# pola-rs/polars

Hardware: AMD Instinct MI355X
Metric: rows/sec + achieved HBM GB/s, TPC-H Q1/Q3 SF100, 1/2/4/8 GPU vs CPU (higher is better)
Workload: dtype f64; 1 GPU; tpch_q1_sf100; rows_per_gpu=600000000, algorithmic_bytes_per_gpu_step=25200000000, parallelism=single GPU

## Files before the change

### include/polars_amd.h

```cpp
#ifndef POLARS_AMD_H
#define POLARS_AMD_H

#include <stddef.h>
#include <stdint.h>

#ifdef __cplusplus
extern "C" {
#endif

#define PLX_ABI_MAJOR 0
#define PLX_ABI_MINOR 1

#define PLX_OK 0
#define PLX_ERR_INVALID 1
#define PLX_ERR_HIP 2
#define PLX_ERR_UNSUPPORTED 3
#define PLX_ERR_OOM 4
#define PLX_ERR_SHAPE 5
#define PLX_ERR_NOT_FOUND 6
#define PLX_ERR_CANCELLED 7

typedef enum plx_dtype {
  PLX_BOOL = 0,
  PLX_I8 = 1,
// ... 213 lines not shown
  PLX_AE_BITMAP_LOOKUP = 12,
  PLX_AE_TEMPORAL = 13,
  PLX_AE_WINDOW = 14,
  PLX_AE_WINDOW_KEY = 15,
  PLX_AE_CUMULATIVE = 16,
  PLX_AE_RANK = 17
} plx_aexpr_kind;

typedef enum plx_operator {
  PLX_OP_EQ = 0, PLX_OP_NE = 1, PLX_OP_LT = 2, PLX_OP_LE = 3, PLX_OP_GT = 4, PLX_OP_GE = 5,
  PLX_OP_PLUS = 6, PLX_OP_MINUS = 7, PLX_OP_MULTIPLY = 8, PLX_OP_TRUE_DIVIDE = 9,
  PLX_OP_FLOOR_DIVIDE = 10, PLX_OP_MODULUS = 11, PLX_OP_AND = 12, PLX_OP_OR = 13, PLX_OP_XOR = 14
} plx_operator;

typedef struct plx_aexpr {
  int32_t kind;
  int32_t op;
  int32_t lhs;
  int32_t rhs;
  int32_t dtype;
  int32_t is_null;
  plx_scalar lit;
  const char* name;
  int32_t cond;
} plx_aexpr;

typedef enum plx_ir_kind {
  PLX_IR_SCAN = 0,
  PLX_IR_FILTER = 1,
  PLX_IR_SELECT = 2,
  PLX_IR_HSTACK = 3,
  PLX_IR_GROUPBY = 4,
  PLX_IR_JOIN = 5,
  PLX_IR_SORT = 6,
  PLX_IR_SLICE = 7,
  PLX_IR_DISTINCT = 8
} plx_ir_kind;

typedef enum plx_join_order {
  PLX_JOIN_ORDER_NONE = 0,
  PLX_JOIN_ORDER_LEFT = 1,
  PLX_JOIN_ORDER_RIGHT = 2,
  PLX_JOIN_ORDER_LEFT_RIGHT = 3,
  PLX_JOIN_ORDER_RIGHT_LEFT = 4
} plx_join_order;

typedef struct plx_ir {
  int32_t kind;
  int32_t input;
  int32_t input_right;
  int32_t predicate;
  plx_frame frame;
  const int32_t* exprs;
  int32_t n_exprs;
  const int32_t* keys;
  int32_t n_keys;
  const int32_t* keys_right;
  int32_t n_keys_right;
  int32_t how;
  int32_t maintain_order;
  const char* suffix;
  const uint8_t* sort_descending;
  const uint8_t* sort_nulls_last;
  int64_t slice_offset;
  int64_t slice_len;
  int32_t coalesce;
} plx_ir;

#define PLX_PLAN_NO_FUSION 1u
#define PLX_PLAN_NO_PARTITION 4u
#define PLX_PLAN_NO_DIRECT_JOIN 2u

int plx_execute_plan(const plx_ir* ir, int32_t n_ir, const plx_aexpr* exprs, int32_t n_exprs, int32_t root,
                     uint32_t flags, plx_frame* out);
int plx_describe_fusion(const plx_ir* ir, int32_t n_ir, const plx_aexpr* exprs, int32_t n_exprs, int32_t root, int32_t* fusable,
                        int32_t* static_shape_id, char* why_not, size_t why_cap);
int plx_debug_program_json(const plx_ir* ir, int32_t n_ir, const plx_aexpr* exprs, int32_t n_exprs, int32_t root, char* buf, size_t cap);
int plx_jit_selftest(const plx_ir* ir, int32_t n_ir, const plx_aexpr* exprs, int32_t n_exprs, int32_t root);
int plx_jit_stats(int32_t* compiled, double* compile_ms);
int plx_jit_set_min_rows(int64_t min_rows);
const char* plx_last_plan_description(void);
const char* plx_last_plan_encodings(void);
int32_t plx_last_scan_tile_rows(void);
int32_t plx_wide_tiles_choice(int32_t compiled, int32_t knob_on, int64_t n_rows, int32_t n_inputs, const int32_t* dtypes, const int32_t* nullable, const uint64_t* values,
                              const uint64_t* validity);

int plx_datagen_lineitem_q1(int64_t n_rows, uint64_t seed, plx_column* out_cols);
int plx_datagen_lineitem_q1_host(int64_t row0, int64_t n, uint64_t seed, int64_t* shipdate, uint8_t* returnflag, uint8_t* linestatus,
                                 int64_t* quantity, double* extendedprice, double* discount, double* tax);

int plx_datagen_orders_lineitem(int64_t n_orders, uint64_t seed, plx_column* out_orders, plx_column* out_lineitem);
int plx_datagen_orders_lineitem_host(int64_t order0, int64_t n, int64_t n_orders_total, uint64_t seed, int64_t* orderkey, int64_t* custkey,
                                     int64_t* orderdate, uint32_t* n_lines, int64_t line_cap, int64_t* l_orderkey, double* l_extendedprice,
                                     double* l_discount, int64_t* l_shipdate, int64_t* n_lines_out);
int plx_datagen_customer(int64_t n_customers, uint64_t seed, plx_column* out_cols);
int plx_datagen_customer_host(int64_t row0, int64_t n, uint64_t seed, int64_t* custkey, uint8_t* segment);
int plx_datagen_uniform(int32_t dtype, int64_t n_rows, uint64_t seed, uint32_t stream, int64_t lo, int64_t hi, double scale, plx_column* out);
int plx_datagen_uniform_host(int32_t dtype, int64_t row0, int64_t n, uint64_t seed, uint32_t stream, int64_t lo, int64_t hi, double scale, void* out);
int plx_datagen_zipf(int64_t n_rows, uint64_t seed, uint32_t stream, uint64_t x0_q62, int64_t n_keys, plx_column* out);
int plx_datagen_zipf_host(int64_t row0, int64_t n, uint64_t seed, uint32_t stream, uint64_t x0_q62, int64_t n_keys, int64_t* out);

typedef uint64_t plx_strdict;
int plx_strview_dict_encode(const void* views, const uint8_t* validity, int64_t bit_offset, int64_t n, const void* const* data_buffers, const int64_t* data_sizes,
                            int32_t n_data_buffers, plx_column* out_codes, plx_strdict* out_dict);
int plx_strview_dict_encode_device(plx_column views_u64_pairs, plx_column data_u8, plx_column* out_codes, plx_strdict* out_dict);
int plx_strview_stamp_nulls(plx_column views_u64_pairs, plx_column valid_bool);
int plx_strview_groupby(plx_column views_u64_pairs, plx_column value, plx_column* out_codes, plx_strdict* out_dict, plx_column* out_sum, plx_column* out_count, plx_column* out_len);
#define PLX_STR_MATCH_MAX_PATTERN 64
typedef enum plx_str_match_kind { PLX_STR_STARTS_WITH = 0, PLX_STR_ENDS_WITH = 1, PLX_STR_CONTAINS = 2 } plx_str_match_kind;
int plx_strdict_match(plx_strdict dict, int32_t kind, const uint8_t* pattern, int64_t pattern_len, plx_column* out_bool);
int plx_strview_match(plx_column views_u64_pairs, plx_column data_u8, int32_t kind, const uint8_t* pattern, int64_t pattern_len, plx_column* out_bool);
int plx_strview_match_host(const void* views, const uint8_t* data, int64_t data_len, int64_t n, int32_t kind, const uint8_t* pattern, int64_t pattern_len,
                           uint64_t* out_bits, uint64_t* out_valid);
int plx_bitmap_lookup(plx_column codes, plx_column lut_bool, plx_column* out_bool);
int plx_strdict_info(plx_strdict dict, int64_t* n_strings, int64_t* total_bytes);

typedef enum plx_time_unit { PLX_UNIT_DATE = 0, PLX_UNIT_MS = 1, PLX_UNIT_US = 2, PLX_UNIT_NS = 3 } plx_time_unit;
typedef enum plx_temporal_part_kind {
  PLX_PART_YEAR = 0, PLX_PART_MONTH = 1, PLX_PART_DAY = 2, PLX_PART_QUARTER = 3, PLX_PART_WEEKDAY = 4, PLX_PART_ORDINAL_DAY = 5,
  PLX_PART_HOUR = 6, PLX_PART_MINUTE = 7, PLX_PART_SECOND = 8, PLX_PART_DATE = 9
} plx_temporal_part_kind;
int plx_temporal_part(plx_column col, int part, int unit, plx_column* out);
int plx_temporal_part_host(const void* values, int unit, int part, int64_t n, void* out);

int plx_strdict_to_host(plx_strdict dict, int64_t* offsets, uint8_t* bytes);
int plx_strdict_free(plx_strdict dict);
int plx_datagen_id_views(int64_t n_rows, uint64_t seed, uint32_t stream, int64_t lo, int64_t hi, plx_column* out_views);
int plx_datagen_long_id_views(int64_t n_rows, uint64_t seed, uint32_t stream, int64_t lo, int64_t hi, plx_column* out_views, plx_column* out_data);

typedef uint64_t plx_parquet;
int plx_parquet_open(const char* path, plx_parquet* out);
int plx_parquet_close(plx_parquet file);
int plx_parquet_shape(plx_parquet file, int64_t* num_rows, int32_t* num_row_groups, int32_t* num_columns);
int plx_parquet_column_info(plx_parquet file, int32_t column, const char** name, int32_t* dtype, int32_t* logical, int32_t* nullable);
int plx_parquet_column_timezone(plx_parquet file, int32_t column, const char** timezone);
int plx_parquet_row_group_info(plx_parquet file, int32_t row_group, int64_t* num_rows, int64_t* compressed_bytes);
int plx_parquet_chunk_info(plx_parquet file, int32_t row_group, int32_t column, int32_t* codec, uint32_t* encodings, int64_t* compressed_bytes,
                           int64_t* uncompressed_bytes, int32_t* has_min_max, plx_scalar* min, plx_scalar* max, int64_t* null_count);
int plx_parquet_read(plx_parquet file, const int32_t* row_groups, int32_t n_row_groups, const int32_t* columns, int32_t n_columns, plx_frame* out);
int plx_parquet_categories(plx_parquet file, int32_t column, int64_t* n_strings, int64_t* total_bytes);
int plx_parquet_categories_to_host(plx_parquet file, int32_t column, int64_t* offsets, uint8_t* bytes);
int plx_parquet_column_strdict(plx_parquet file, int32_t column, plx_strdict* out);

typedef uint64_t plx_ipc;
int plx_ipc_open(const char* path, plx_ipc* out);
int plx_ipc_close(plx_ipc file);
int plx_ipc_shape(plx_ipc file, int64_t* num_rows, int32_t* num_batches, int32_t* num_columns);
int plx_ipc_column_info(plx_ipc file, int32_t column, const char** name, int32_t* dtype, int32_t* logical, int32_t* nullable);
int plx_ipc_column_timezone(plx_ipc file, int32_t column, const char** timezone);
int plx_ipc_batch_info(plx_ipc file, int32_t batch, int64_t* num_rows, int64_t* body_bytes, int32_t* compressed);
int plx_ipc_read(plx_ipc file, const int32_t* batches, int32_t n_batches, const int32_t* columns, int32_t n_columns, plx_frame* out);
int plx_ipc_read_string_views(plx_ipc file, const int32_t* batches, int32_t n_batches, int32_t column, plx_column* out_views, plx_column* out_data);
int plx_ipc_categories(plx_ipc file, int32_t column, int64_t* n_strings, int64_t* total_bytes);
int plx_ipc_categories_to_host(plx_ipc file, int32_t column, int64_t* offsets, uint8_t* bytes);
int plx_ipc_column_strdict(plx_ipc file, int32_t column, plx_strdict* out);

typedef uint64_t plx_comm;
int plx_comm_unique_id(uint8_t* out_128_bytes);
int plx_comm_init(const uint8_t* unique_id_128_bytes, int32_t rank, int32_t world_size, plx_comm* out);
int plx_comm_info(plx_comm comm, int32_t* rank, int32_t* world_size);
int plx_comm_free(plx_comm comm);
int plx_exchange_by_key(plx_comm comm, plx_frame frame, const char* key, uint64_t seed, plx_frame* out, uint64_t* rows_sent, uint64_t* bytes_sent);
int plx_allgather_frame(plx_comm comm, plx_frame frame, plx_frame* out);

typedef struct plx_profile_record {
  char name[48];
// ... 43 lines not shown
```

### polars_amd/_ffi.py

```python
from __future__ import annotations

import ctypes as C
import os
import threading
from typing import Optional

os.environ.setdefault("GPU_MAX_HW_QUEUES", "8")

_HERE = os.path.dirname(os.path.abspath(__file__))
LIB_PATH = os.path.join(_HERE, "libpolars_amd.so")

BOOL, I8, I16, I32, I64, U8, U16, U32, U64, F32, F64 = range(11)
EQ, NE, LT, LE, GT, GE = range(6)
ADD, SUB, MUL, TRUE_DIV, FLOOR_DIV, MOD = range(6)
AND, OR, XOR = range(3)
AGG_SUM, AGG_MEAN, AGG_MIN, AGG_MAX, AGG_COUNT, AGG_LEN, AGG_FIRST, AGG_VAR, AGG_STD = range(9)
AGG_QUANTILE = 9
AGG_N_UNIQUE = 10
UNIQUE_ANY, UNIQUE_FIRST, UNIQUE_LAST, UNIQUE_NONE = range(4)
UNIQUE_KEEPS = {"any": UNIQUE_ANY, "first": UNIQUE_FIRST, "last": UNIQUE_LAST, "none": UNIQUE_NONE}
QUANTILE_NEAREST, QUANTILE_LOWER, QUANTILE_HIGHER, QUANTILE_MIDPOINT, QUANTILE_LINEAR = range(5)
QUANTILE_INTERPOLATIONS = {"nearest": QUANTILE_NEAREST, "lower": QUANTILE_LOWER, "higher": QUANTILE_HIGHER, "midpoint": QUANTILE_MIDPOINT, "linear": QUANTILE_LINEAR}
JOIN_INNER, JOIN_LEFT, JOIN_SEMI, JOIN_ANTI, JOIN_FULL, JOIN_RIGHT = range(6)
JOIN_COALESCE_DEFAULT, JOIN_COALESCE, JOIN_KEEP_BOTH = range(3)
# ... 134 lines not shown
    "plx_parquet_chunk_info": (C.c_int, [C.c_uint64, C.c_int32, C.c_int32, _i32p, C.POINTER(C.c_uint32), _i64p, _i64p, _i32p, C.POINTER(Scalar), C.POINTER(Scalar), _i64p]),
    "plx_parquet_read": (C.c_int, [C.c_uint64, _i32p, C.c_int32, _i32p, C.c_int32, _u64p]),
    "plx_parquet_categories": (C.c_int, [C.c_uint64, C.c_int32, _i64p, _i64p]),
    "plx_parquet_categories_to_host": (C.c_int, [C.c_uint64, C.c_int32, C.c_void_p, C.c_void_p]),
    "plx_parquet_column_strdict": (C.c_int, [C.c_uint64, C.c_int32, _u64p]),
    "plx_ipc_open": (C.c_int, [C.c_char_p, _u64p]),
    "plx_ipc_close": (C.c_int, [C.c_uint64]),
    "plx_ipc_shape": (C.c_int, [C.c_uint64, _i64p, _i32p, _i32p]),
    "plx_ipc_column_info": (C.c_int, [C.c_uint64, C.c_int32, C.POINTER(C.c_char_p), _i32p, _i32p, _i32p]),
    "plx_ipc_column_timezone": (C.c_int, [C.c_uint64, C.c_int32, C.POINTER(C.c_char_p)]),
    "plx_ipc_batch_info": (C.c_int, [C.c_uint64, C.c_int32, _i64p, _i64p, _i32p]),
    "plx_ipc_read": (C.c_int, [C.c_uint64, _i32p, C.c_int32, _i32p, C.c_int32, _u64p]),
    "plx_ipc_read_string_views": (C.c_int, [C.c_uint64, _i32p, C.c_int32, C.c_int32, _u64p, _u64p]),
    "plx_ipc_categories": (C.c_int, [C.c_uint64, C.c_int32, _i64p, _i64p]),
    "plx_ipc_categories_to_host": (C.c_int, [C.c_uint64, C.c_int32, C.c_void_p, C.c_void_p]),
    "plx_ipc_column_strdict": (C.c_int, [C.c_uint64, C.c_int32, _u64p]),
    "plx_comm_unique_id": (C.c_int, [C.c_void_p]),
    "plx_comm_init": (C.c_int, [C.c_void_p, C.c_int32, C.c_int32, _u64p]),
    "plx_comm_info": (C.c_int, [C.c_uint64, C.POINTER(C.c_int32), C.POINTER(C.c_int32)]),
    "plx_comm_free": (C.c_int, [C.c_uint64]),
    "plx_exchange_by_key": (C.c_int, [C.c_uint64, C.c_uint64, C.c_char_p, C.c_uint64, _u64p, _u64p, _u64p]),
    "plx_allgather_frame": (C.c_int, [C.c_uint64, C.c_uint64, _u64p]),
    "plx_column_import_arrow": (C.c_int, [C.POINTER(ArrowArray), C.POINTER(ArrowSchema), _u64p]),
    "plx_column_import_series": (C.c_int, [C.POINTER(SeriesExport), _u64p]),
    "plx_column_export_arrow": (C.c_int, [C.c_uint64, C.POINTER(ArrowArray), C.POINTER(ArrowSchema)]),
    "plx_column_export_series": (C.c_int, [C.c_uint64, C.c_char_p, C.POINTER(SeriesExport)]),
    "plx_column_to_host": (C.c_int, [C.c_uint64, C.c_void_p, C.c_void_p, _i32p]),
    "plx_column_copy_to_device": (C.c_int, [C.c_uint64, C.c_void_p, C.c_void_p]),
    "plx_column_info": (C.c_int, [C.c_uint64, _i32p, _i64p, _i64p]),
    "plx_column_device_ptrs": (C.c_int, [C.c_uint64, C.POINTER(C.c_void_p), C.POINTER(C.c_void_p)]),
    "plx_column_retain": (C.c_int, [C.c_uint64]),
    "plx_column_free": (C.c_int, [C.c_uint64]),
    "plx_cmp": (C.c_int, [C.c_int, C.c_uint64, C.c_uint64, _u64p]),
    "plx_cmp_scalar": (C.c_int, [C.c_int, C.c_uint64, Scalar, _u64p]),
    "plx_bitmap_binop": (C.c_int, [C.c_int, C.c_uint64, C.c_uint64, _u64p]),
    "plx_bitmap_not": (C.c_int, [C.c_uint64, _u64p]),
    "plx_arith": (C.c_int, [C.c_int, C.c_uint64, C.c_uint64, _u64p]),
    "plx_arith_scalar": (C.c_int, [C.c_int, C.c_uint64, Scalar, C.c_int, _u64p]),
    "plx_cast": (C.c_int, [C.c_uint64, C.c_int, _u64p]),
    "plx_if_then_else": (C.c_int, [C.c_uint64, C.c_uint64, C.c_uint64, _u64p]),
    "plx_filter": (C.c_int, [C.c_uint64, C.c_uint64, _u64p]),
    "plx_gather": (C.c_int, [C.c_uint64, C.c_uint64, _u64p]),
    "plx_reduce": (C.c_int, [C.c_int, C.c_uint64, C.POINTER(Scalar), _i32p, _i32p]),
    "plx_reduce_var": (C.c_int, [C.c_uint64, C.c_int32, C.c_int32, C.POINTER(Scalar), _i32p, _i32p]),
    "plx_groupby_agg": (C.c_int, [_u64p, C.c_int32, _u64p, _i32p, C.c_int32, C.c_int32, _u64p, _u64p]),
    "plx_groupby_agg_ddof": (C.c_int, [_u64p, C.c_int32, _u64p, _i32p, C.c_int32, C.c_int32, _i32p, _u64p, _u64p]),
    "plx_reduce_quantile": (C.c_int, [C.c_uint64, C.c_double, C.c_int32, C.POINTER(Scalar), _i32p, _i32p]),
    "plx_groupby_agg_params": (C.c_int, [_u64p, C.c_int32, _u64p, _i32p, C.c_int32, C.c_int32, _i32p, C.POINTER(C.c_double), _i32p, _u64p, _u64p]),
    "plx_window_agg": (C.c_int, [_u64p, C.c_int32, _u64p, _i32p, C.c_int32, _i32p, C.POINTER(C.c_double), _i32p, _u64p]),
    "plx_cumulative": (C.c_int, [_u64p, C.c_int32, C.c_uint64, C.c_int32, C.c_int32, _u64p]),
    "plx_rank": (C.c_int, [_u64p, C.c_int32, C.c_uint64, C.c_int32, C.c_int32, _u64p]),
    "plx_join_indices": (C.c_int, [C.c_int, C.c_uint64, C.c_uint64, _u64p, _u64p]),
    "plx_datagen_lineitem_q1": (C.c_int, [C.c_int64, C.c_uint64, _u64p]),
    "plx_datagen_lineitem_q1_host": (C.c_int, [C.c_int64, C.c_int64, C.c_uint64, C.c_void_p, C.c_void_p, C.c_void_p, C.c_void_p, C.c_void_p, C.c_void_p, C.c_void_p]),
    "plx_datagen_orders_lineitem": (C.c_int, [C.c_int64, C.c_uint64, _u64p, _u64p]),
    "plx_datagen_orders_lineitem_host": (C.c_int, [C.c_int64, C.c_int64, C.c_int64, C.c_uint64, C.c_void_p, C.c_void_p, C.c_void_p, C.c_void_p, C.c_int64,
                                                   C.c_void_p, C.c_void_p, C.c_void_p, C.c_void_p, _i64p]),
    "plx_datagen_uniform": (C.c_int, [C.c_int32, C.c_int64, C.c_uint64, C.c_uint32, C.c_int64, C.c_int64, C.c_double, _u64p]),
    "plx_datagen_customer": (C.c_int, [C.c_int64, C.c_uint64, _u64p]),
    "plx_datagen_customer_host": (C.c_int, [C.c_int64, C.c_int64, C.c_uint64, C.c_void_p, C.c_void_p]),
    "plx_datagen_uniform_host": (C.c_int, [C.c_int32, C.c_int64, C.c_int64, C.c_uint64, C.c_uint32, C.c_int64, C.c_int64, C.c_double, C.c_void_p]),
    "plx_datagen_zipf": (C.c_int, [C.c_int64, C.c_uint64, C.c_uint32, C.c_uint64, C.c_int64, _u64p]),
    "plx_datagen_zipf_host": (C.c_int, [C.c_int64, C.c_int64, C.c_uint64, C.c_uint32, C.c_uint64, C.c_int64, C.c_void_p]),
    "plx_debug_program_json": (C.c_int, [C.POINTER(IR), C.c_int32, C.POINTER(AExpr), C.c_int32, C.c_int32, C.c_char_p, C.c_size_t]),
    "plx_reduce_n_unique": (C.c_int, [C.c_uint64, C.POINTER(C.c_uint32)]),
    "plx_distinct_mask": (C.c_int, [_u64p, C.c_int32, C.c_int32, _u64p]),
    "plx_sort_indices": (C.c_int, [_u64p, C.c_int32, C.POINTER(C.c_uint8), C.POINTER(C.c_uint8), C.c_int64, _u64p]),
    "plx_hash_partition": (C.c_int, [C.c_uint64, C.c_int32, C.c_uint64, _u64p, _i64p]),
    "plx_frame_new": (C.c_int, [C.POINTER(C.c_char_p), _u64p, C.c_int32, _u64p]),
    "plx_frame_free": (C.c_int, [C.c_uint64]),
    "plx_frame_concat": (C.c_int, [_u64p, C.c_int32, _u64p]),
    "plx_frame_shape": (C.c_int, [C.c_uint64, _i64p, _i32p]),
    "plx_frame_column": (C.c_int, [C.c_uint64, C.c_int32, C.POINTER(C.c_char_p), _u64p]),
    "plx_frame_dtypes": (C.c_int, [C.c_uint64, _i32p]),
    "plx_frame_to_host": (C.c_int, [C.c_uint64, C.POINTER(C.c_void_p), C.POINTER(C.c_void_p), _i32p]),
    "plx_execute_plan": (C.c_int, [C.POINTER(IR), C.c_int32, C.POINTER(AExpr), C.c_int32, C.c_int32, C.c_uint32, _u64p]),
    "plx_describe_fusion": (C.c_int, [C.POINTER(IR), C.c_int32, C.POINTER(AExpr), C.c_int32, C.c_int32, _i32p, _i32p, C.c_char_p, C.c_size_t]),
    "plx_jit_selftest": (C.c_int, [C.POINTER(IR), C.c_int32, C.POINTER(AExpr), C.c_int32, C.c_int32]),
    "plx_jit_stats": (C.c_int, [_i32p, C.POINTER(C.c_double)]),
    "plx_jit_set_min_rows": (C.c_int, [C.c_int64]),
    "plx_last_plan_description": (C.c_char_p, []),
    "plx_last_plan_encodings": (C.c_char_p, []),
    "plx_last_scan_tile_rows": (C.c_int32, []),
    "plx_wide_tiles_choice": (C.c_int32, [C.c_int32, C.c_int32, C.c_int64, C.c_int32, C.POINTER(C.c_int32), C.POINTER(C.c_int32), C.POINTER(C.c_uint64), C.POINTER(C.c_uint64)]),
    "plx_profile_enable": (C.c_int, [C.c_int]),
    "plx_profile_fetch": (C.c_int, [C.POINTER(ProfileRecord), C.c_int32, _i32p]),
    "plx_profile_clear": (C.c_int, []),
}

_lib: Optional[C.CDLL] = None


def lib() -> C.CDLL:
    global _lib
    if _lib is None:
        if not os.path.exists(LIB_PATH):
            raise ImportError(
                f"{LIB_PATH} is missing: build the HIP extension first "
                "(python -c 'import __graft_entry__ as g; g.build()' or make -C polars_amd/csrc). "
                "There is no CPU fallback in polars_amd.")
        l = C.CDLL(LIB_PATH, mode=C.RTLD_GLOBAL)
        for name, (res, args) in SIGNATURES.items():
            fn = getattr(l, name)
            fn.restype = res
            fn.argtypes = args
        _lib = l
    return _lib


def check(status: int) -> None:
    if status != 0:
        msg = lib().plx_last_error().decode("utf-8", "replace")
        if status == ERR_UNSUPPORTED:
            raise UnsupportedError(status, msg)
        raise PlxError(status, msg)


_initialised = False


def init(device: Optional[int] = None) -> None:
    global _initialised
    if device is None:
        device = int(os.environ.get("LOCAL_RANK", "0"))
    check(lib().plx_init(device))
    _initialised = True


def ensure_init() -> None:
    if not _initialised:
        init()


_tls = threading.local()


def set_plan_note(note) -> None:
    _tls.plan_note = note


def last_plan() -> str:
    note = getattr(_tls, "plan_note", None)
    return note if note is not None else lib().plx_last_plan_description().decode()


def last_plan_encodings() -> str:
    return lib().plx_last_plan_encodings().decode()


def last_scan_tile_rows() -> int:
    return int(lib().plx_last_scan_tile_rows())


def wide_tiles_choice(compiled, knob_on, n_rows, dtypes, nullable, values, validity) -> int:
    n = len(dtypes)
    return int(lib().plx_wide_tiles_choice(int(bool(compiled)), int(bool(knob_on)), int(n_rows), n, (C.c_int32 * n)(*[int(d) for d in dtypes]),
                                           (C.c_int32 * n)(*[int(bool(x)) for x in nullable]), (C.c_uint64 * n)(*[int(v) for v in values]), (C.c_uint64 * n)(*[int(v) for v in validity])))


def jit_set_min_rows(min_rows: int) -> None:
    check(lib().plx_jit_set_min_rows(int(min_rows)))


def encoded_set_decimal_min_rows(min_rows: int) -> None:
    check(lib().plx_encoded_set_decimal_min_rows(int(min_rows)))


def encoded_decimal_min_rows() -> int:
    return int(lib().plx_encoded_decimal_min_rows())


def jit_stats():
    n, ms = C.c_int32(), C.c_double()
    check(lib().plx_jit_stats(C.byref(n), C.byref(ms)))
    return n.value, ms.value
```

### polars_amd/csrc/abi.cpp

```cpp
#include <cstdio>
#include <cstring>
#include <memory>
#include <mutex>

#include "core.hpp"
#include "datagen_device.hpp"
#include "distinct.hpp"
#include "encoded_inputs.hpp"
#include "engine.hpp"
#include "fused_shapes.hpp"
#include "jit.hpp"
#include "join.hpp"
#include "kernels.hpp"
#include "kernels_fused.hpp"
#include "ops.hpp"
#include "cumulative.hpp"
#include "quantile.hpp"
#include "scan.hpp"
#include "sort.hpp"
#include "strmatch.hpp"
#include "temporal.hpp"

namespace plx {
void init_device(int ordinal);
// ... 1115 lines not shown
    if (n_lines) n_lines[j] = r.n_lines;
    const bool want_lines = l_orderkey || l_extendedprice || l_discount || l_shipdate;
    for (uint32_t q = 0; q < r.n_lines; q++, at++) {
      if (!want_lines) continue;
      PLX_REQUIRE(at < line_cap, PLX_ERR_INVALID, "datagen: line arrays too small");
      const datagen::Q3LineRow lr = datagen::q3_line_row(seed, (uint64_t)(order0 + j), q, r.orderdate);
      if (l_orderkey) l_orderkey[at] = r.orderkey;
      if (l_extendedprice) l_extendedprice[at] = lr.extendedprice;
      if (l_discount) l_discount[at] = lr.discount;
      if (l_shipdate) l_shipdate[at] = lr.shipdate;
    }
  }
  if (n_lines_out) *n_lines_out = at;
  PLX_CATCH
}
int plx_datagen_customer(int64_t n_customers, uint64_t seed, plx_column* out_cols) {
  PLX_TRY
  PLX_REQUIRE(n_customers >= 0 && out_cols, PLX_ERR_INVALID, "datagen: bad arguments");
  ColumnPtr k = make_column(PLX_I64, n_customers, false), sgm = make_column(PLX_U8, n_customers, false);
  k->null_count = 0; sgm->null_count = 0;
  k::datagen_customer(n_customers, seed, k->values->as<int64_t>(), sgm->values->as<uint8_t>());
  out_cols[0] = register_column(k); out_cols[1] = register_column(sgm);
  PLX_CATCH
}
int plx_datagen_customer_host(int64_t row0, int64_t n, uint64_t seed, int64_t* custkey, uint8_t* segment) {
  PLX_TRY
  PLX_REQUIRE(row0 >= 0 && n >= 0, PLX_ERR_INVALID, "datagen: bad arguments");
  for (int64_t j = 0; j < n; j++) {
    if (custkey) custkey[j] = row0 + j + 1;
    if (segment) segment[j] = datagen::customer_segment(seed, (uint64_t)(row0 + j + 1));
  }
  PLX_CATCH
}
int plx_datagen_uniform(int32_t dtype, int64_t n_rows, uint64_t seed, uint32_t stream_id, int64_t lo, int64_t hi, double scale, plx_column* out) {
  PLX_TRY
  PLX_REQUIRE(n_rows >= 0 && out && hi > lo && stream_id < 8, PLX_ERR_INVALID, "datagen: bad arguments");
  PLX_REQUIRE(dtype == PLX_I64 || dtype == PLX_U32 || dtype == PLX_F64, PLX_ERR_UNSUPPORTED, "datagen_uniform: dtype must be Int64, UInt32 or Float64");
  ColumnPtr c = make_column(dtype, n_rows, false); c->null_count = 0;
  k::datagen_uniform(dtype, n_rows, seed, stream_id, lo, hi, scale, c->values->ptr);
  *out = register_column(c);
  PLX_CATCH
}
int plx_datagen_uniform_host(int32_t dtype, int64_t row0, int64_t n, uint64_t seed, uint32_t stream_id, int64_t lo, int64_t hi, double scale, void* out) {
  PLX_TRY
  PLX_REQUIRE(row0 >= 0 && n >= 0 && (out || n == 0) && hi > lo && stream_id < 8, PLX_ERR_INVALID, "datagen: bad arguments");
  PLX_REQUIRE(dtype == PLX_I64 || dtype == PLX_U32 || dtype == PLX_F64, PLX_ERR_UNSUPPORTED, "datagen_uniform: dtype must be Int64, UInt32 or Float64");
  for (int64_t j = 0; j < n; j++) {
    const int64_t v = datagen::uniform_value(seed, stream_id, (uint64_t)(row0 + j), lo, hi);
    if (dtype == PLX_I64) reinterpret_cast<int64_t*>(out)[j] = v;
    else if (dtype == PLX_U32) reinterpret_cast<uint32_t*>(out)[j] = (uint32_t)v;
    else reinterpret_cast<double*>(out)[j] = (double)v * scale;
  }
  PLX_CATCH
}

int plx_datagen_zipf(int64_t n_rows, uint64_t seed, uint32_t stream_id, uint64_t x0_q62, int64_t n_keys, plx_column* out) {
  PLX_TRY
  PLX_REQUIRE(n_rows >= 0 && out && n_keys > 0 && stream_id < 8 && x0_q62 > 0 && x0_q62 < (1ull << 62), PLX_ERR_INVALID, "datagen_zipf: bad arguments");
  ColumnPtr c = make_column(PLX_I64, n_rows, false); c->null_count = 0;
  k::datagen_zipf(n_rows, seed, stream_id, x0_q62, n_keys, c->values->as<int64_t>());
  *out = register_column(c);
  PLX_CATCH
}
int plx_datagen_zipf_host(int64_t row0, int64_t n, uint64_t seed, uint32_t stream_id, uint64_t x0_q62, int64_t n_keys, int64_t* out) {
  PLX_TRY
  PLX_REQUIRE(row0 >= 0 && n >= 0 && (out || n == 0) && n_keys > 0 && stream_id < 8 && x0_q62 > 0 && x0_q62 < (1ull << 62), PLX_ERR_INVALID, "datagen_zipf: bad arguments");
  for (int64_t j = 0; j < n; j++) out[j] = datagen::zipf_value(seed, stream_id, (uint64_t)(row0 + j), x0_q62, n_keys);
  PLX_CATCH
}

int plx_execute_plan(const plx_ir* ir, int32_t n_ir, const plx_aexpr* exprs, int32_t n_exprs, int32_t root, uint32_t flags, plx_frame* out) {
  PLX_TRY
  PLX_REQUIRE(out, PLX_ERR_INVALID, "null out pointer");
  engine::Plan p = engine::import_plan(ir, n_ir, exprs, n_exprs, flags);
  FramePtr f = engine::execute(p, root);
  t_plan_desc = p.desc;
  t_plan_encoded = p.encoded;
  *out = register_frame(f);
  PLX_CATCH
}
const char* plx_last_plan_description(void) { return t_plan_desc.c_str(); }
const char* plx_last_plan_encodings(void) { return t_plan_encoded.c_str(); }
int32_t plx_last_scan_tile_rows(void) { return k::last_scan_tile_rows(); }
int32_t plx_wide_tiles_choice(int32_t compiled, int32_t knob_on, int64_t n_rows, int32_t n_inputs, const int32_t* dtypes, const int32_t* nullable, const uint64_t* values,
                              const uint64_t* validity) {
  if (n_inputs < 0 || n_inputs > fused::kMaxInputs || (n_inputs && (!dtypes || !nullable || !values || !validity))) return -1;
  fused::Shape sh{}; fused::Args args{};
  sh.n_inputs = (uint8_t)n_inputs; sh.pred = fused::kNone; sh.key = fused::kNone;
  args.n_rows = n_rows;
  for (int i = 0; i < n_inputs; i++) {
    sh.in_dtype[i] = (uint8_t)dtypes[i]; sh.in_nullable[i] = (uint8_t)(nullable[i] != 0);
    args.in[i].values = (const void*)(uintptr_t)values[i]; args.in[i].validity = (const uint64_t*)(uintptr_t)validity[i];
  }
  return k::wide_tiles_choice(sh, args, compiled != 0, knob_on != 0) ? 1 : 0;
}

int plx_debug_program_json(const plx_ir* ir, int32_t n_ir, const plx_aexpr* exprs, int32_t n_exprs, int32_t root, char* buf, size_t cap) {
  PLX_TRY
  PLX_REQUIRE(buf && cap > 0, PLX_ERR_INVALID, "null buffer");
  engine::Plan p = engine::import_plan(ir, n_ir, exprs, n_exprs, 0);
  std::string json, why;
  if (!engine::dump_program_json(p, root, &json, &why)) fail(PLX_ERR_UNSUPPORTED, "not a fusable pipeline: " + why);
  PLX_REQUIRE(json.size() + 1 <= cap, PLX_ERR_INVALID, "buffer too small for the program dump (" + std::to_string(json.size() + 1) + " bytes)");
  memcpy(buf, json.c_str(), json.size() + 1);
  PLX_CATCH
}

int plx_describe_fusion(const plx_ir* ir, int32_t n_ir, const plx_aexpr* exprs, int32_t n_exprs, int32_t root, int32_t* fusable, int32_t* static_shape_id,
                        char* why_not, size_t why_cap) {
  PLX_TRY
  engine::Plan p = engine::import_plan(ir, n_ir, exprs, n_exprs, 0);
  auto dump = [](const fused::Shape& sh) {
    std::string d = "inputs=" + std::to_string(sh.n_inputs) + " pred=" + std::to_string(sh.pred) + " key=" + std::to_string(sh.key) + " ops=[";
    for (int i = 0; i < sh.n_ops; i++) d += "(" + std::to_string(sh.ops[i].code) + "," + std::to_string(sh.ops[i].dst) + "," + std::to_string(sh.ops[i].a) + "," + std::to_string(sh.ops[i].b) + "," + std::to_string(sh.ops[i].c) + ")";
    d += "] aggs=[";
    for (int i = 0; i < sh.n_aggs; i++) d += "(" + std::to_string(sh.aggs[i].kind) + "," + std::to_string(sh.aggs[i].src) + ")";
    d += "] in_dtype=[";
    for (int i = 0; i < sh.n_inputs; i++) d += std::to_string(sh.in_dtype[i]) + (sh.in_nullable[i] ? "?" : "") + ",";
    d += "]";
    if (sh.n_keys) { d += " keys=["; for (int i = 0; i < sh.n_keys; i++) d += std::to_string(sh.keys[i]) + ","; d += "]"; }
    return d;
  };
  std::string why;
  int sid = -1;
  bool ok;
  PLX_REQUIRE(root >= 0 && root < (int)p.ir.size(), PLX_ERR_INVALID, "bad root");
  const engine::IRN& rn = p.ir[root];
  if (rn.kind == PLX_IR_GROUPBY && rn.input >= 0 && p.ir[rn.input].kind == PLX_IR_JOIN) {
    std::vector<fused::Shape> shapes;
    ok = engine::describe_join_fusion(p, root, &shapes, &why);
    if (ok) {
      sid = fused::find_static_shape(shapes[2]);
      t_plan_desc = dump(shapes[0]);
      for (size_t i = 1; i < shapes.size(); i++) t_plan_desc += "\n" + dump(shapes[i]);
    }
  } else {
    fused::Shape sh{};
    ok = engine::describe_fusion(p, root, &sh, &sid, &why);
    if (ok) t_plan_desc = dump(sh);
  }
  if (fusable) *fusable = ok ? 1 : 0;
  if (static_shape_id) *static_shape_id = sid;
  if (why_not && why_cap) snprintf(why_not, why_cap, "%s", why.c_str());
  PLX_CATCH
}

int plx_jit_selftest(const plx_ir* ir, int32_t n_ir, const plx_aexpr* exprs, int32_t n_exprs, int32_t root) {
  PLX_TRY
  engine::Plan p = engine::import_plan(ir, n_ir, exprs, n_exprs, 0);
  PLX_REQUIRE(root >= 0 && root < (int)p.ir.size(), PLX_ERR_INVALID, "bad root");
  const engine::IRN& rn = p.ir[root];
  std::string why;
  std::vector<std::pair<fused::Shape, jit::Sink>> jobs;
  if (rn.kind == PLX_IR_GROUPBY && rn.input >= 0 && p.ir[rn.input].kind == PLX_IR_JOIN) {
    std::vector<fused::Shape> shapes;
    PLX_REQUIRE(engine::describe_join_fusion(p, root, &shapes, &why), PLX_ERR_UNSUPPORTED, "not fusable: " + why);
    jobs = {{shapes[0], jit::REGAGG}, {shapes[1], jit::JOIN_BUILD}, {shapes[1], jit::DIRECT_BUILD}, {shapes[2], jit::PROBE_AGG}, {shapes[2], jit::DIRECT_PROBE}};
    for (size_t i = 3; i + 1 < shapes.size(); i++) jobs.push_back({shapes[i], jit::BITMAP_BUILD});
    for (uint32_t tiles : {2u, 4u}) jobs.push_back({shapes.back(), jit::part3_scatter_sink(fused::kP2Direct, tiles, fused::kPackRowid, false)});
  } else if (rn.kind == PLX_IR_FILTER) {
    fused::Shape sh{};
    PLX_REQUIRE(engine::describe_filter_fusion(p, root, &sh, &why), PLX_ERR_UNSUPPORTED, "not fusable: " + why);
    jobs = {{sh, jit::BALLOT}};
  } else {
    fused::Shape sh{}; int sid = -1;
    PLX_REQUIRE(engine::describe_fusion(p, root, &sh, &sid, &why), PLX_ERR_UNSUPPORTED, "not fusable: " + why);
    if (rn.kind == PLX_IR_SELECT) jobs = {{sh, jit::REGAGG}};
    else jobs = {{sh, jit::LDSAGG}, {sh, jit::DENSE}, {sh, jit::HASH}, {sh, jit::PART_COUNT}, {sh, jit::PART_SCATTER}, {sh, jit::PART_AGG},
                  {sh, jit::PART2_SCATTER_HASH}, {sh, jit::PART2_SCATTER_DIRECT}, {sh, jit::PART2_AGG_HASH}, {sh, jit::PART2_AGG_DIRECT},
                  {sh, jit::PART2_SCATTER_HASH_T2}, {sh, jit::PART2_SCATTER_DIRECT_T2}};
    if (rn.kind != PLX_IR_SELECT && sh.n_keys < 2) {
      for (uint32_t mode = 0; mode < 2; mode++) {
        const uint32_t best = fused::best_static_pack(sh, mode);
        for (uint32_t pack = 0; pack <= best; pack++) {
          if (pack == fused::kPackNarrow && fused::rec_layout2(sh, mode, fused::kPackNarrow).rec_words == fused::rec_layout2(sh, mode, fused::kPackNone).rec_words) continue;
          for (uint32_t tiles : {1u, 2u, 3u, 4u}) { jobs.push_back({sh, jit::part3_scatter_sink(mode, tiles, pack, false)}); jobs.push_back({sh, jit::part3_scatter_sink(mode, tiles, pack, true)}); }
          jobs.push_back({sh, jit::part3_agg_sink(mode, pack)});
        }
      }
      for (uint32_t mode = 0; mode < 2; mode++) {
        if (!fused::pair_pack_ok(sh, mode)) continue;
        for (uint32_t tiles : {1u, 2u, 3u, 4u}) { if (mode == fused::kP2Hash && tiles > 3) continue; jobs.push_back({sh, jit::part3_scatter_sink(mode, tiles, fused::kPackPair, false)}); jobs.push_back({sh, jit::part3_scatter_sink(mode, tiles, fused::kPackPair, true)}); }
        jobs.push_back({sh, jit::part3_agg_sink(mode, fused::kPackPair)});
      }
      if (fused::pairv_pack_ok(sh, fused::kP2Hash)) {
        for (uint32_t tiles : {1u, 2u, 3u}) { jobs.push_back({sh, jit::part3_scatter_sink(fused::kP2Hash, tiles, fused::kPackPairV, false)}); jobs.push_back({sh, jit::part3_scatter_sink(fused::kP2Hash, tiles, fused::kPackPairV, true)}); }
        jobs.push_back({sh, jit::part3_agg_sink(fused::kP2Hash, fused::kPackPairV)});
      }
    }
    if (sh.n_keys >= 2) {
      jobs = {{sh, jit::WIDE}};
      for (uint32_t pack = 0; pack <= std::min<uint32_t>(fused::best_static_pack(sh, fused::kP2Hash), fused::kPackNarrow); pack++) {
        for (uint32_t tiles : {1u, 2u, 3u}) jobs.push_back({sh, jit::part3_scatter_sink(fused::kP2Hash, tiles, pack, false)});
        jobs.push_back({sh, jit::part3_agg_sink(fused::kP2Hash, pack)});
      }
    }
  }
  {
    std::vector<std::pair<fused::Shape, jit::Sink>> forms;
    fused::Args aligned{}; aligned.n_rows = fused::kWideTileRows;
    for (auto& j : jobs) {
      const bool wide = k::wide_tiles_choice(j.first, aligned, true, true);
      if (j.second == jit::REGAGG && wide) forms.push_back({j.first, jit::REGAGG_WIDE});
      if (j.second == jit::LDSAGG && wide) forms.push_back({j.first, jit::LDSAGG_WIDE});
    }
    jobs.insert(jobs.end(), forms.begin(), forms.end());
  }
  for (auto& j : jobs) {
    const std::string log = jit::selftest(j.first, j.second);
    if (!log.empty()) fail(PLX_ERR_INVALID, "jit selftest failed: " + log.substr(0, 4000));
  }
  PLX_CATCH
}
int plx_jit_set_min_rows(int64_t min_rows) { PLX_TRY jit::set_min_rows(min_rows); PLX_CATCH }
int plx_jit_stats(int32_t* compiled, double* compile_ms) {
  PLX_TRY
  int c = 0; double ms = 0;
  jit::stats(&c, &ms);
  if (compiled) *compiled = c;
  if (compile_ms) *compile_ms = ms;
  PLX_CATCH
}

extern "C++" {
namespace {
struct StrDict { Buf views, data, offsets, bytes; int64_t n = 0; uint64_t total = 0; bool materialised = false; };
std::mutex g_strdict_mu;
std::vector<std::unique_ptr<StrDict>> g_strdicts;
StrDict& get_strdict(uint64_t h) {
  std::lock_guard<std::mutex> lk(g_strdict_mu);
  if (h == 0 || h > g_strdicts.size() || !g_strdicts[h - 1]) fail(PLX_ERR_INVALID, "invalid string dictionary handle");
  return *g_strdicts[h - 1];
}
uint64_t register_strdict(std::unique_ptr<StrDict> d) { std::lock_guard<std::mutex> lk(g_strdict_mu); g_strdicts.push_back(std::move(d)); return (uint64_t)g_strdicts.size(); }
void materialise(StrDict& d) {
  if (d.materialised) return;
  k::strdict_materialise(d.views->as<uint64_t>(), d.data ? d.data->as<uint8_t>() : nullptr, d.n, &d.offsets, &d.bytes, &d.total);
  d.materialised = true;
}
void encode_on_device(const uint64_t* views, const ColumnPtr& validity_holder, Buf data, Buf buf_base, int64_t n, plx_column* out_codes, plx_strdict* out_dict, bool from_stamps = false) {
  Buf codes, dviews, svalid;
  int64_t nd = 0, snulls = 0;
  k::strview_dict_encode(views, validity_holder ? validity_holder->valid_words() : nullptr, data ? data->as<uint8_t>() : nullptr, buf_base ? buf_base->as<uint64_t>() : nullptr, n, &codes, &dviews, &nd,
                         from_stamps && !validity_holder ? &svalid : nullptr, &snulls);
  auto c = std::make_shared<Column>();
  c->dtype = PLX_U32; c->len = n; c->values = codes;
  if (validity_holder && validity_holder->validity) c->validity = validity_holder->validity;
  else if (snulls > 0) { c->validity = svalid; c->null_count = snulls; }
  else c->null_count = 0;
  if (nd > 0) { c->range_state = 1; c->range_min = 0; c->range_max = nd - 1; c->range_trusted = true; }
  auto d = std::make_unique<StrDict>();
  d->views = dviews; d->data = data; d->n = nd;
  *out_codes = register_column(c);
  *out_dict = register_strdict(std::move(d));
}
}
namespace plx {
void strview_encode_device(const uint64_t* views, const ColumnPtr& validity_holder, Buf data, int64_t n, plx_column* out_codes, plx_strdict* out_dict) {
  Buf bb = dev_alloc_zero(8);
  encode_on_device(views, validity_holder, data, bb, n, out_codes, out_dict);
}
void strview_encode_device_bases(const uint64_t* views, const ColumnPtr& validity_holder, Buf data, Buf buf_base, int64_t n, plx_column* out_codes, plx_strdict* out_dict) {
  encode_on_device(views, validity_holder, data, buf_base, n, out_codes, out_dict);
}
}
}

int plx_strview_dict_encode(const void* views, const uint8_t* validity, int64_t bit_offset, int64_t n, const void* const* data_buffers, const int64_t* data_sizes,
                            int32_t n_data_buffers, plx_column* out_codes, plx_strdict* out_dict) {
  PLX_TRY
  PLX_REQUIRE(out_codes && out_dict && n >= 0 && (views || n == 0) && n_data_buffers >= 0 && (n_data_buffers == 0 || (data_buffers && data_sizes)), PLX_ERR_INVALID, "strview_dict_encode: bad arguments");
  device();
  Buf dv = dev_alloc((size_t)std::max<int64_t>(n, 1) * 16);
  if (n) h2d_sync_pinned(dv->ptr, views, (size_t)n * 16);
  ColumnPtr vh;
  if (validity) {
    std::vector<uint8_t> zeros((size_t)n);
    vh = column_from_host(PLX_U8, zeros.data(), validity, bit_offset, n);
  }
  uint64_t total = 0;
  std::vector<uint64_t> base((size_t)std::max(n_data_buffers, 1), 0);
  for (int i = 0; i < n_data_buffers; i++) { base[i] = total; total += (uint64_t)data_sizes[i]; }
  Buf data = dev_alloc((size_t)total + 64), bb = dev_alloc(sizeof(uint64_t) * base.size());
  for (int i = 0; i < n_data_buffers; i++) {
    if (!data_sizes[i]) continue;
    if ((uint64_t)data_sizes[i] >= ((uint64_t)32 << 20)) h2d_sync_pinned((uint8_t*)data->ptr + base[i], data_buffers[i], (size_t)data_sizes[i]);
    else h2d_async((uint8_t*)data->ptr + base[i], data_buffers[i], (size_t)data_sizes[i]);
  }
  h2d_async(bb->ptr, base.data(), sizeof(uint64_t) * base.size());
  PLX_HIP(hipStreamSynchronize(stream()));
  encode_on_device(dv->as<uint64_t>(), vh, data, bb, n, out_codes, out_dict);
  PLX_CATCH
}
// ... 242 lines not shown
```

### polars_amd/csrc/engine.cpp

```cpp
#include "engine.hpp"

#include <algorithm>
#include <atomic>
#include <cmath>
#include <functional>
#include <memory>
#include <numeric>
#include <optional>
#include <set>
#include <sstream>

#include "cumulative.hpp"
#include "distinct.hpp"
#include "encoded_inputs.hpp"
#include "fused_shapes.hpp"
#include "jit.hpp"
#include "join.hpp"
#include "kernels.hpp"
#include "kernels_fused.hpp"
#include "ops.hpp"
#include "quantile.hpp"
#include "sort.hpp"
#include "temporal.hpp"
#include "variance.hpp"
// ... 1208 lines not shown
  }
  int64_t mn, mx;
  if (col->range_state == 1 && col->range_trusted && !col->range_assumed) { mn = col->range_min; mx = col->range_max; }
  else {
    const k::ReduceResult rr = k::reduce_all(col->dtype, col->data(), col->valid_words(), n);
    if (rr.n_valid == 0) return nullptr;
    mn = (int64_t)rr.minmax_lo; mx = (int64_t)rr.minmax_hi;
  }
  uint64_t g = 0;
  if (enc::affine_needs_gcd(mn, mx)) {
    if (col->dtype != PLX_I64) return nullptr;
    g = enc::affine_gcd(col->values->as<int64_t>(), col->valid_words(), n, mn);
  }
  const enc::AffineChoice ch = enc::choose_affine(mn, mx, g);
  if (!ch.ok || ch.width * 4 > dtype_width(col->dtype)) return nullptr;
  s->kind = EncodedShadow::kAffine; s->width = ch.width; s->base = ch.base; s->stride = ch.stride;
  s->codes = dev_alloc(groups * (size_t)ch.width);
  if (!enc::affine_encode(col->dtype, col->data(), col->valid_words(), n, ch.base, ch.stride, ch.width, s->codes->ptr)) return nullptr;
  return s;
}
static std::shared_ptr<EncodedShadow> encoded_shadow_for_scan(const ColumnPtr& col, bool may_build) {
  if (!encoded_inputs_enabled()) return nullptr;
  std::shared_ptr<EncodedShadow> s = std::atomic_load(&col->shadow);
  if (s && s->kind != EncodedShadow::kNone) return s;
  if (!may_build || (s && s->never_encode) || !col->values || !col->values->owned || col->len <= 0) return nullptr;
  if (col->dtype != PLX_I64 && col->dtype != PLX_F64 && col->dtype != PLX_I32 && col->dtype != PLX_U32) return nullptr;
  auto next = std::make_shared<EncodedShadow>();
  next->scans = (s ? s->scans : 0) + 1;
  if (next->scans >= 2) {
    std::shared_ptr<EncodedShadow> built;
    try { built = build_shadow(col); }
    catch (const Error& e) { if (e.code != PLX_ERR_OOM) throw; (void)hipGetLastError(); }
    if (built) { built->scans = next->scans; next = built; }
    else next->never_encode = true;
  }
  std::atomic_store(&col->shadow, next);
  return next->kind != EncodedShadow::kNone ? next : nullptr;
}
struct ScanProgram { Shape shape; Args args; int static_id; std::string note; };
static ScanProgram scan_program_with_encodings(const Compiler& c, bool may_build) {
  ScanProgram sp{c.shape, c.args, -1, ""};
  enc::InputEncoding e[kMaxInputs];
  bool any = false;
  for (int i = 0; i < c.shape.n_inputs; i++) {
    const ColumnPtr& col = c.cols[c.input_cols[i]];
    if (c.args.in[i].values != col->data() || c.args.n_rows != col->len) continue;
    const std::shared_ptr<EncodedShadow> s = encoded_shadow_for_scan(col, may_build);
    if (!s) continue;
    e[i].kind = s->kind; e[i].width = s->width; e[i].base = s->base; e[i].stride = s->stride;
    e[i].codes = s->codes ? s->codes->ptr : nullptr; e[i].dict = s->dict ? s->dict->as<unsigned long long>() : nullptr;
    any = true;
  }
  uint32_t taken = 0;
  if (any && enc::encode_program(c.shape, c.args, e, &sp.shape, &sp.args, &taken)) {
    sp.note = "encoded{";
    bool first = true;
    for (int i = 0; i < c.shape.n_inputs; i++) {
      if (!((taken >> i) & 1u)) continue;
      std::string name = "?";
      for (size_t j = 0; j < c.df->cols.size(); j++) if (c.df->cols[j] == c.cols[c.input_cols[i]]) name = c.df->names[j];
      sp.note += std::string(first ? "" : ",") + name + ":" + (e[i].kind == EncodedShadow::kDict ? "dict" : e[i].kind == EncodedShadow::kDecimal ? "decimal" : "affine") + std::to_string(8 * e[i].width);
      first = false;
    }
    sp.note += "}";
  }
  sp.static_id = find_static_shape(sp.shape);
  return sp;
}

namespace {
struct GroupByRun {
  Compiler& c; const KeyPlan& kp; const Shape& sh; const Args& args;
  const int len_idx, static_id;
  const bool may_partition;
  FusedAggResult& res; std::string& desc;
};
std::string scan_tag(int static_id, int64_t n_rows) { return std::string("fused_scan[") + jit::program_mode(static_id, n_rows) + "]+"; }

void finish_table(GroupByRun& q, const Buf& cells, int64_t G, const Buf& oob) {
  compact_into(nullptr, cells->as<uint64_t>(), G, -1, q.sh.n_aggs, q.len_idx, q.res);
  check_oob_flag(oob);
  q.res.key_valid = nullptr;
}
void lds_table(GroupByRun& q) {
  const int G = 1 << q.kp.total_bits;
  Buf cells = dev_alloc(sizeof(uint64_t) * (size_t)G * q.sh.n_aggs);
  Buf oob = untrusted_key_bounds(q.c) ? dev_alloc_zero(8) : nullptr;
  k::fused_lds_agg(q.sh, q.args, G, q.static_id, cells->as<uint64_t>(), oob ? oob->as<unsigned int>() : nullptr);
  q.desc += scan_tag(q.static_id, q.args.n_rows) + "lds_table(G=" + std::to_string(G) + ",copies=" + std::to_string(k::lds_agg_copies(G, q.sh.n_aggs)) + ")";
  finish_table(q, cells, G, oob);
}
void dense_hbm_table(GroupByRun& q) {
  const int64_t G = (int64_t)1 << q.kp.total_bits;
  Buf cells = dev_alloc(sizeof(uint64_t) * (size_t)(G + 1) * q.sh.n_aggs);
  k::init_agg_cells(cells->as<uint64_t>(), G + 1, q.sh);
  Buf oob = untrusted_key_bounds(q.c) ? dev_alloc_zero(8) : nullptr;
  DenseTable t; t.acc = cells->as<unsigned long long>(); t.key_min = 0; t.n_groups = G; t.oob = oob ? oob->as<unsigned int>() : nullptr;
  k::fused_dense_agg(q.sh, q.args, t, q.static_id);
  q.desc += scan_tag(q.static_id, q.args.n_rows) + "dense_hbm_table(G=" + std::to_string(G) + ")";
  finish_table(q, cells, G, oob);
}

enum PartKeys { kPackedIds , kKeysWithValidity, kWideWords };
void take_partitioned(GroupByRun& q, PartKeys keys, int64_t g, const Buf& ok, const Buf& okv, const Buf& oacc, int64_t stride, const std::string& pd) {
  FusedAggResult& res = q.res;
  res.n_groups = g; res.n_aggs = q.sh.n_aggs; res.acc = oacc;
  if (keys == kWideWords) { res.wide_words = ok; res.wide_valid = okv; res.wide_stride = stride; }
  else { res.packed_keys = ok; res.key_valid = keys == kKeysWithValidity ? okv : nullptr; }
  q.desc += scan_tag(q.static_id, q.args.n_rows) + pd;
}
bool partitioned_v1(GroupByRun& q, double est_groups, bool any_nullable, PartKeys keys) {
  PartitionPlan pp;
  if (!k::partition_plan(q.sh, est_groups, any_nullable, &pp)) return false;
  std::string pd;
  Buf ok, okv, oacc;
  const int64_t g = k::partitioned_agg(q.sh, q.args, pp, q.static_id, &ok, &okv, &oacc, &pd);
  if (g < 0) { q.desc += "lds-overflow+"; return false; }
  take_partitioned(q, keys, g, ok, okv, oacc, 0, pd);
  return true;
}
struct PartTry {
  double plan_for = 0;
  double fallback = 0;
  int packed_bits = -1;
  std::vector<uint64_t> hot;
  k::SrcRange ranges[kMaxSrc];
  k::SrcRange key_rng;
  ColumnPtr stat_col;
  int attempts = 3;
  bool grow_to_largest = false;
  PartKeys keys = kPackedIds;
};
bool partitioned_v2(GroupByRun& q, PartTry& t) {
  for (int attempt = 0; attempt < t.attempts; attempt++) {
    PartPlan2 p2;
    auto plan = [&](double groups) { return k::partition_plan2(q.sh, groups, t.packed_bits, q.len_idx, q.args.n_rows, (int)t.hot.size(), &p2, t.ranges, &t.key_rng); };
    if (!plan(t.plan_for) && !(attempt == 0 && t.fallback > 0 && plan(t.fallback))) return false;
    std::string pd;
    Buf ok, okv, oacc;
    int64_t key_range[2] = {1, 0}, stride = 0;
    const int64_t g = k::partitioned_agg2(q.sh, q.args, p2, q.static_id, t.hot, &ok, &okv, &oacc, &pd, t.stat_col ? key_range : nullptr, &stride);
    if (g >= 0) {
      if (t.stat_col && key_range[0] <= key_range[1]) { t.stat_col->range_state = 1; t.stat_col->range_min = key_range[0]; t.stat_col->range_max = key_range[1]; t.stat_col->range_trusted = true; pd += "+key_range_learned"; }
      if (p2.check_src) mark_sources_verified(q.c);
      if (t.keys == kKeysWithValidity) q.desc += "hot=" + std::to_string(t.hot.size()) + "+";
      take_partitioned(q, t.keys, g, ok, okv, oacc, stride, pd);
      return true;
    }
    if (g == -2) { q.desc += "v2-unavailable+"; return false; }
    q.desc += t.attempts == 1 ? "lds-overflow+" : "lds-overflow(P=" + std::to_string(1u << p2.log2_parts) + ")+";
    if (p2.log2_parts >= 9) return false;
    t.plan_for = std::max(t.plan_for * 2.0, t.grow_to_largest ? (double)((uint64_t)p2.n_slots << 9) * 0.8 : (double)((uint64_t)p2.n_slots << p2.log2_parts) * 1.01);
  }
  return false;
}

bool partitioned_packed_ids(GroupByRun& q) {
  const int bits = q.kp.total_bits;
  const int64_t n = q.args.n_rows;
  const double est = std::min((double)((uint64_t)1 << std::min(bits, 40)), (double)n);
  if (part_version() != 2) return partitioned_v1(q, est, false, kPackedIds);
  PartTry t;
  t.plan_for = est; t.packed_bits = bits; t.attempts = 1;
  if (hot_keys_enabled() || bits > 25) {
    double g_est = 1e18;
    const int64_t d = sample_keys_cached(plain_key_column(q.c, q.kp), q.sh, q.args, q.static_id, q.len_idx, kPartSampleRows, hot_keys_enabled() ? &t.hot : nullptr, &g_est, q.desc);
    if (d >= 0) t.plan_for = std::min(est, std::min(g_est, (double)n) * 1.3);
    q.desc += "sample(distinct=" + std::to_string(d) + ",hot=" + std::to_string(t.hot.size()) + ")+";
  }
  const double hint = q.c.plan.group_hint;
  if (hint > 0) { t.plan_for = std::min(est, hint * 1.02 + 64.0); q.desc += "groups<=" + std::to_string((int64_t)hint) + "(plan)+"; }
// ... 2118 lines not shown
```

### polars_amd/csrc/fused_sinks.hpp

```cpp
#pragma once
#include <type_traits>

#include "fused_device.hpp"

namespace plx {
namespace k {

struct RegAggSink {
  struct Params { unsigned long long* partials; };
  uint64_t acc[kMaxAggs];
  template <class S> __device__ __forceinline__ void init(const S& sh, const Params&) {
#pragma unroll
    for (int k = 0; k < kMaxAggs; k++) acc[k] = (k < sh.n_aggs) ? agg_identity_dev(sh.aggs[k].kind) : 0ull;
  }
  template <class S, class RF> __device__ __forceinline__ void consume(const S& sh, const RF& rf, const bool pass[kRows], int64_t row0, const Params&) {
#pragma unroll
    for (int r = 0; r < kRows; r++) {
#pragma unroll
      for (int k = 0; k < kMaxAggs; k++) {
        if (k < sh.n_aggs) {
          const Agg ag = sh.aggs[k];
          uint64_t v = rf.get(r, ag.src);
          bool valid = (rf.getv(ag.src) >> r) & 1;
          acc[k] = agg_combine(ag.kind, acc[k], agg_row_value(ag.kind, v, pass[r], valid, (uint64_t)(row0 + r)));
        }
      }
    }
  }
  template <class S> __device__ __forceinline__ void finish(const S& sh, const Params& p) {
    __shared__ uint64_t sh_acc[kBlock / 64][kMaxAggs];
    const int lane = lane_id(), wave = threadIdx.x >> 6;
#pragma unroll
    for (int k = 0; k < kMaxAggs; k++) {
      if (k < sh.n_aggs) {
        uint64_t x = acc[k];
#pragma unroll
        for (int m = 32; m >= 1; m >>= 1) x = agg_combine(sh.aggs[k].kind, x, shfl_xor_u64(x, m));
        if (lane == 0) sh_acc[wave][k] = x;
      }
    }
    __syncthreads();
    if ((int)threadIdx.x < sh.n_aggs) {
      const int k = threadIdx.x;
      uint64_t x = sh_acc[0][k];
      for (int w = 1; w < (int)(blockDim.x >> 6); w++) x = agg_combine(sh.aggs[k].kind, x, sh_acc[w][k]);
      p.partials[(size_t)blockIdx.x * kMaxAggs + k] = x;
    }
  }
};

struct LdsAggSink {
  struct Params {
    unsigned long long* partials;
    unsigned long long* global_acc;
    int n_groups;
    int copies;
    unsigned int* oob;
  };
  template <class S> __device__ __forceinline__ void init(const S& sh, const Params& p) {
    extern __shared__ unsigned long long lds_tbl[];
    const int cells = p.n_groups * sh.n_aggs;
    for (int i = threadIdx.x; i < cells * p.copies; i += blockDim.x) lds_tbl[i] = agg_identity_dev(sh.aggs[(i / p.copies) % sh.n_aggs].kind);
    __syncthreads();
  }
  template <class S, class RF> __device__ __forceinline__ void consume(const S& sh, const RF& rf, const bool pass[kRows], int64_t row0, const Params& p) {
    extern __shared__ unsigned long long lds_tbl[];
    const int copy = lane_id() & (p.copies - 1);
#pragma unroll
    for (int r = 0; r < kRows; r++) {
      if (!pass[r]) continue;
      const uint64_t gid64 = rf.get(r, sh.key);
      if (gid64 >= (uint64_t)p.n_groups) { if (p.oob) *p.oob = 1u; continue; }
      const uint32_t gid = (uint32_t)gid64;
      unsigned long long* cells = lds_tbl + (size_t)gid * sh.n_aggs * p.copies + copy;
#pragma unroll
      for (int k = 0; k < kMaxAggs; k++) {
        if (k < sh.n_aggs) {
          const Agg ag = sh.aggs[k];
          uint64_t v = rf.get(r, ag.src);
          bool valid = (rf.getv(ag.src) >> r) & 1;
          if ((ag.kind == AGG_SUM_F || ag.kind == AGG_SUM_I || ag.kind == AGG_COUNT) && !valid) continue;
          uint64_t x = agg_row_value(ag.kind, v, true, valid, (uint64_t)(row0 + r));
          lds_atomic_agg(ag.kind, cells + k * p.copies, x);
        }
      }
    }
  }
  template <class S> __device__ __forceinline__ void finish(const S& sh, const Params& p) {
    extern __shared__ unsigned long long lds_tbl[];
    __syncthreads();
    const int cells = p.n_groups * sh.n_aggs;
    for (int i = threadIdx.x; i < cells; i += blockDim.x) {
      const uint8_t kind = sh.aggs[i % sh.n_aggs].kind;
      uint64_t x = lds_tbl[(size_t)i * p.copies];
      for (int c = 1; c < p.copies; c++) x = agg_combine(kind, x, lds_tbl[(size_t)i * p.copies + c]);
      if (p.global_acc) { if (x != agg_identity_dev(kind) || kind == AGG_SUM_F) atomic_agg(kind, p.global_acc + i, x); }
      else p.partials[(size_t)blockIdx.x * cells + i] = x;
    }
  }
};

struct DenseAggSink {
  using Params = DenseTable;
  template <class S> __device__ __forceinline__ void init(const S&, const Params&) {}
  template <class S> __device__ __forceinline__ void finish(const S&, const Params&) {}
  template <class S, class RF> __device__ __forceinline__ void consume(const S& sh, const RF& rf, const bool pass[kRows], int64_t row0, const Params& p) {
#pragma unroll
    for (int r = 0; r < kRows; r++) {
      if (!pass[r]) continue;
      bool kvalid = (rf.getv(sh.key) >> r) & 1;
      int64_t g = kvalid ? ((int64_t)rf.get(r, sh.key) - p.key_min) : p.n_groups;
      if ((uint64_t)g > (uint64_t)p.n_groups || (kvalid && g == p.n_groups)) { if (p.oob) *p.oob = 1u; continue; }
      atomic_row(sh, rf, r, row0 + r, p.acc + (size_t)g * sh.n_aggs);
    }
  }
};

struct HashAggSink {
  using Params = HashTable;
  template <class S> __device__ __forceinline__ void init(const S&, const Params&) {}
  template <class S> __device__ __forceinline__ void finish(const S&, const Params&) {}
  __device__ __forceinline__ static int64_t find_slot(const Params& p, uint64_t key) {
    const uint64_t cap = 1ull << p.log2_cap;
    uint64_t slot = (key * 0x55fbfd6bfc5458e9ull) >> (64 - p.log2_cap);
    for (uint32_t probe = 0; probe < p.max_probe; probe++) {
      unsigned long long cur = p.keys[slot];
      if (cur == key) return (int64_t)slot;
      if (cur == kEmptyKey) {
        unsigned long long old = atomicCAS(&p.keys[slot], (unsigned long long)kEmptyKey, (unsigned long long)key);
        if (old == kEmptyKey || old == key) return (int64_t)slot;
      }
      slot = (slot + 1) & (cap - 1);
    }
    atomicExch(p.overflow, 1u);
    return -1;
  }
  static constexpr int kCombineRounds = 8;
  template <class S, class RF> __device__ __forceinline__ void consume_combined(const S& sh, const RF& rf, const bool pass[kRows], int64_t row0, const Params& p) {
    const uint64_t cap = 1ull << p.log2_cap;
    const int lane = lane_id();
#pragma unroll
    for (int r = 0; r < kRows; r++) {
      const bool kvalid = (rf.getv(sh.key) >> r) & 1;
      const uint64_t key = kvalid ? rf.get(r, sh.key) : 0ull;
      uint64_t xv[kMaxAggs];
#pragma unroll
      for (int k = 0; k < kMaxAggs; k++) {
        xv[k] = 0;
        if (k < sh.n_aggs) { const Agg ag = sh.aggs[k]; xv[k] = agg_row_value(ag.kind, rf.get(r, ag.src), true, (rf.getv(ag.src) >> r) & 1, (uint64_t)(row0 + r)); }
      }
      bool reached = false, keeps_total = false;
      uint64_t todo = ballot(pass[r]);
#pragma unroll 1
      for (int round = 0; round < kCombineRounds && todo; round++) {
        const int leader = (int)__builtin_ctzll(todo);
        const uint64_t lkey = shfl_u64(key, leader);
        const bool lvalid = __shfl((int)kvalid, leader, 64) != 0;
        const bool member = pass[r] && !reached && kvalid == lvalid && key == lkey;
        todo &= ~ballot(member);
#pragma unroll
        for (int k = 0; k < kMaxAggs; k++) {
          if (k < sh.n_aggs) {
            uint64_t x = member ? xv[k] : agg_identity_dev(sh.aggs[k].kind);
#pragma unroll
            for (int m = 32; m >= 1; m >>= 1) x = agg_combine(sh.aggs[k].kind, x, shfl_xor_u64(x, m));
            if (lane == leader) xv[k] = x;
          }
        }
        if (member) reached = true;
        if (lane == leader) keeps_total = true;
      }
      if (!pass[r] || (reached && !keeps_total)) continue;
      int64_t slot;
      if (!kvalid) { slot = (int64_t)cap; p.keys[cap] = 0; }
      else if (key == kEmptyKey) { slot = (int64_t)cap + 1; p.keys[cap + 1] = 0; }
      else slot = find_slot(p, key);
      if (slot < 0) continue;
#pragma unroll
      for (int k = 0; k < kMaxAggs; k++) {
        if (k < sh.n_aggs) {
          const uint8_t kind = sh.aggs[k].kind;
          if (xv[k] != agg_identity_dev(kind) || kind == AGG_SUM_F) atomic_agg(kind, p.acc + (size_t)slot * sh.n_aggs + k, xv[k]);
        }
// ... 238 lines not shown
};

struct BitmapBuildSink {
  using Params = BitmapBuild;
  unsigned long long n = 0;
  template <class S> __device__ __forceinline__ void init(const S&, const Params&) { n = 0; }
  template <class S> __device__ __forceinline__ void finish(const S&, const Params& p) {
    const uint64_t w = wave_sum_u64(n);
    if (lane_id() == 0 && w) atomicAdd(p.count, (unsigned long long)w);
  }
  template <class S, class RF> __device__ __forceinline__ void consume(const S& sh, const RF& rf, const bool pass[kRows], int64_t, const Params& p) {
#pragma unroll
    for (int r = 0; r < kRows; r++) {
      if (!pass[r] || !((rf.getv(sh.key) >> r) & 1)) continue;
      const uint64_t idx = rf.get(r, sh.key) - (uint64_t)p.kmin;
      if (idx >= p.range) continue;
      n++;
      __hip_atomic_fetch_or(&p.bits[idx >> 6], 1ull << (idx & 63), __ATOMIC_RELAXED, __HIP_MEMORY_SCOPE_AGENT);
    }
  }
};

struct DirectHitsSink {
  using Params = DirectHits;
  template <class S> __device__ __forceinline__ void init(const S&, const Params&) {}
  template <class S> __device__ __forceinline__ void finish(const S&, const Params&) {}
  template <class S, class RF> __device__ __forceinline__ void consume(const S& sh, const RF& rf, const bool pass[kRows], int64_t row0, const Params& p) {
    bool hit[kRows];
#pragma unroll
    for (int r = 0; r < kRows; r++) {
      bool ok = pass[r] && ((rf.getv(sh.key) >> r) & 1);
      const uint64_t idx = rf.get(r, sh.key) - (uint64_t)p.t.kmin;
      ok = ok && idx < p.t.range;
      if (ok) ok = (p.t.bits[idx >> 6] >> (idx & 63)) & 1ull;
      hit[r] = ok;
    }
    const unsigned long long b0 = ballot(hit[0]), b1 = ballot(hit[1]);
    if (lane_id() == 0) {
      const int64_t t = row0 / kTileRows;
      *reinterpret_cast<ulonglong2*>(p.out.ballots + t * 2) = make_ulonglong2(b0, b1);
      p.out.counts[t] = (unsigned int)(popc64(b0) + popc64(b1));
    }
  }
};

template <class P, bool FULL>
__device__ __forceinline__ void direct_probe_tile(const Args& args, const DirectJoinTable& p, int64_t base, RegFile& rf) {
  constexpr Shape sh = P::shape();
  const int64_t row0 = base + (int64_t)lane_id() * kRows;
  run_split<P, FULL, true>(args, row0, rf);
  if (!(p.opts & kDirectLateLoads)) run_split<P, FULL, false>(args, row0, rf);
  bool hit[kRows], any = false;
  unsigned long long slot[kRows];
#pragma unroll
  for (int r = 0; r < kRows; r++) {
    bool ok = FULL || (row0 + r < args.n_rows);
    if (sh.pred != kNone) ok = ok && (rf.get(r, sh.pred) & 1) && ((rf.getv(sh.pred) >> r) & 1);
    ok = ok && ((rf.getv(sh.key) >> r) & 1);
    const uint64_t idx = rf.get(r, sh.key) - (uint64_t)p.kmin;
    ok = ok && idx < p.range;
    slot[r] = 0;
    if (ok) {
      const unsigned long long w = p.bits[idx >> 6];
      ok = (w >> (idx & 63)) & 1ull;
      if (ok) slot[r] = direct_slot(p, idx, w);
    }
    hit[r] = ok; any = any || ok;
  }
  if (any) {
    if (p.opts & kDirectLateLoads) run_split<P, FULL, false>(args, row0, rf);
#pragma unroll
    for (int r = 0; r < kRows; r++)
      if (hit[r]) atomic_row(sh, rf, r, row0 + r, p.acc + (size_t)slot[r] * sh.n_aggs);
  }
}

template <class P, class Sink>
__host__ __device__ constexpr bool late_probe() {
  if constexpr (P::kStatic && std::is_same<Sink, DirectProbeAggSink>::value) return split_program(P::shape()).any_late;
  else return false;
}
template <class P, class Sink>
__host__ __device__ constexpr bool trust_nullable() {
  if constexpr (P::kStatic && (std::is_same<Sink, LdsAggSink>::value || std::is_same<Sink, RegAggSink>::value)) return narrow_rows(P::shape());
  else return false;
}
template <class P, class Sink>
__host__ __device__ constexpr bool wide_tiles_form() {
  if constexpr (trust_nullable<P, Sink>()) return wide_tiles_shape(P::shape());
  else return false;
}
template <class P, class Sink, bool WIDE = false>
__device__ __forceinline__ void fused_scan_body(const Shape dsh, const Args args, const typename Sink::Params sp) {
  Sink sink;
  typename RegFileOf<P>::type rf = make_regfile<P>(args);
  const int64_t wave = ((int64_t)blockIdx.x * blockDim.x + threadIdx.x) >> 6;
  const int64_t nwaves = ((int64_t)gridDim.x * blockDim.x) >> 6;
  const int64_t ntiles = (args.n_rows + kTileRows - 1) / kTileRows;
  if constexpr (late_probe<P, Sink>()) {
    for (int64_t t = wave; t < ntiles; t += nwaves) {
      const int64_t base = t * kTileRows;
      if (base + kTileRows <= args.n_rows) direct_probe_tile<P, true>(args, sp, base, rf);
      else direct_probe_tile<P, false>(args, sp, base, rf);
    }
  } else if constexpr (P::kStatic) {
    constexpr Shape sh = P::shape();
    constexpr int ND = dict_count(sh);
    constexpr bool kTrust = trust_nullable<P, Sink>();
    if constexpr (ND > 0) { stage_dicts<ND>(args); __syncthreads(); }
    sink.init(sh, sp);
    int64_t first_tile = 0;
    if constexpr (WIDE) {
      static_assert(wide_tiles_form<P, Sink>(), "wide tiles: a compiled aggregate scan over narrow rows without nullable inputs");
      const int64_t nwide = args.n_rows / kWideTileRows;
      const int lane = lane_id();
      for (int64_t t = wave; t < nwide; t += nwaves) {
        const int64_t row0 = t * kWideTileRows + (int64_t)lane * kWideRows;
        WideRaw raw;
        wide_load<P>(args, row0, raw);
#pragma unroll
        for (int j = 0; j < kWideRows / kRows; j++) {
          run_program_wide<P, ND>(args, raw, j, rf);
          bool pass[kRows];
#pragma unroll
          for (int r = 0; r < kRows; r++) pass[r] = sh.pred == kNone || ((rf.get(r, sh.pred) & 1) && ((rf.getv(sh.pred) >> r) & 1));
          sink.consume(sh, rf, pass, row0 + kRows * j, sp);
        }
      }
      first_tile = nwide * (kWideTileRows / kTileRows);
    }
    for (int64_t t = first_tile + wave; t < ntiles; t += nwaves) {
      bool pass[kRows]; int64_t row0;
      tile_rows<P, ND, kTrust>(dsh, args, t, rf, pass, row0);
      sink.consume(sh, rf, pass, row0, sp);
    }
    sink.finish(sh, sp);
  } else {
    sink.init(dsh, sp);
    for (int64_t t = wave; t < ntiles; t += nwaves) {
      bool pass[kRows]; int64_t row0;
      tile_rows<P>(dsh, args, t, rf, pass, row0);
      sink.consume(dsh, rf, pass, row0, sp);
    }
    sink.finish(dsh, sp);
  }
}

template <class P, class Sink>
__global__ __launch_bounds__(kBlock) void fused_scan_kernel(Shape dsh, Args args, typename Sink::Params sp) {
  fused_scan_body<P, Sink>(dsh, args, sp);
}
template <class P, class Sink>
__global__ __launch_bounds__(kBlock) void fused_scan_wide_kernel(Shape dsh, Args args, typename Sink::Params sp) {
  fused_scan_body<P, Sink, true>(dsh, args, sp);
}

struct BallotSink {
  using Params = BallotOut;
  template <class S> __device__ __forceinline__ void init(const S&, const Params&) {}
  template <class S> __device__ __forceinline__ void finish(const S&, const Params&) {}
  template <class S, class RF> __device__ __forceinline__ void consume(const S&, const RF&, const bool pass[kRows], int64_t row0, const Params& p) {
    const unsigned long long b0 = ballot(pass[0]), b1 = ballot(pass[1]);
    if (lane_id() == 0) {
      const int64_t t = row0 / kTileRows;
      *reinterpret_cast<ulonglong2*>(p.ballots + t * 2) = make_ulonglong2(b0, b1);
      p.counts[t] = (unsigned int)(popc64(b0) + popc64(b1));
    }
// ... 6 lines not shown
```

### polars_amd/csrc/jit.cpp

```cpp
#include "jit.hpp"

#include <dlfcn.h>
#include <sys/stat.h>
#include <unistd.h>
#include <hip/hip_runtime_api.h>
#include <hip/hiprtc.h>

#include <atomic>
#include <chrono>
#include <cstdlib>
#include <cstring>
#include <map>
#include <mutex>
#include <sstream>
#include <string>
#include <vector>

#include "core.hpp"
#include "kconfig.hpp"

namespace plx {
namespace jit {

using namespace fused;

namespace {
struct Entry { hipModule_t mod = nullptr; hipFunction_t fn = nullptr; bool failed = false; };
std::mutex g_mu;
std::map<std::string, Entry> g_cache;
int g_compiled = 0;
double g_ms = 0;

bool wide_tiles(Sink s) { return s == REGAGG_WIDE || s == LDSAGG_WIDE; }
const char* sink_type(Sink s) {
  static const char* n[] = {"RegAggSink", "LdsAggSink", "DenseAggSink", "HashAggSink", "WideAggSink", "JoinBuildSink", "ProbeAggSink", "DirectBuildSink", "DirectProbeAggSink", "BitmapBuildSink",
                            "part_count", "part_scatter", "part_agg", "part2_scatter_hash", "part2_scatter_direct", "part2_agg_hash", "part2_agg_direct", "part2_scatter_hash_t2", "part2_scatter_direct_t2"};
  if (s == REGAGG_WIDE) return "RegAggSink";
  if (s == LDSAGG_WIDE) return "LdsAggSink";
  if (s == PART3_AGG_PAIRV) return "part3_agg";
  if (s >= PART3_SCATTER_PAIRV && s < PART3_AGG_PAIRV) return "part3_scatter";
  if (s == PART3_AGG_PAIR || s == PART3_AGG_PAIR_DIRECT) return "part3_agg";
  if (s >= PART3_SCATTER_PAIR && s < PART3_AGG_PAIR) return "part3_scatter";
  if (s == BALLOT) return "BallotSink";
  if (s == DIRECT_HITS) return "DirectHitsSink";
  if (s >= PART3_AGG) return "part3_agg";
  if (s >= PART3_SCATTER) return "part3_scatter";
  return n[s];
}

std::string include_dir() {
  if (const char* e = getenv("PLX_JIT_INCLUDE")) return e;
  Dl_info info;
  if (dladdr((const void*)&stats, &info) && info.dli_fname) {
    std::string p = info.dli_fname;
    size_t k = p.rfind('/');
    return (k == std::string::npos ? std::string(".") : p.substr(0, k)) + "/csrc";
  }
  return "polars_amd/csrc";
}

std::string resource_include() {
  if (const char* e = getenv("PLX_JIT_CLANG_INCLUDE")) return e;
  const char* roots[] = {"/opt/rocm/lib/llvm/lib/clang", "/opt/rocm/llvm/lib/clang"};
  for (const char* r : roots) {
    for (int v = 30; v >= 14; v--) {
      const std::string p = std::string(r) + "/" + std::to_string(v) + "/include";
      if (FILE* f = fopen((p + "/stddef.h").c_str(), "r")) { fclose(f); return p; }
    }
  }
  return "/opt/rocm/lib/llvm/lib/clang/22/include";
}
std::vector<std::string> compile_options() {
  std::vector<std::string> o = {"--offload-arch=gfx950", "-O3", "-std=c++17", "-ffp-contract=off", "-munsafe-fp-atomics", "-Wno-pass-failed", "-ffreestanding",
                                "-I" + include_dir(), "-I/opt/rocm/include", "-I" + resource_include()};
  if (const char* e = getenv("PLX_JIT_DEFINES")) { std::istringstream is(e); std::string t; while (is >> t) if (t.compare(0, 2, "-D") == 0) o.push_back(t); }
  return o;
}

uint64_t fnv1a(const std::string& s, uint64_t h = 0xcbf29ce484222325ull) { for (unsigned char c : s) { h ^= c; h *= 0x100000001b3ull; } return h; }

std::string kernel_symbol(const Shape& sh, Sink sink) {
  std::string key((const char*)&sh, sizeof(Shape));
  key.push_back((char)sink);
  char out[96];
  snprintf(out, sizeof out, "plx_jit_%s_%d_%08x", sink_type(sink), (int)sink, (unsigned)(fnv1a(key) & 0xffffffffu));
  return out;
}

std::string source_for(const Shape& sh, Sink sink) {
  std::ostringstream o;
  const std::string sym = kernel_symbol(sh, sink);
  o << "#define plx_jit_kernel " << sym << "\n";
  o << ((sink == BALLOT || sink == DIRECT_HITS || wide_tiles(sink)) ? "#include \"fused_sinks.hpp\"\n" : sink >= PART3_SCATTER ? "#include \"partition3_device.hpp\"\n" : sink >= PART2_SCATTER_HASH ? "#include \"partition2_device.hpp\"\n" : sink >= PART_COUNT ? "#include \"partition_device.hpp\"\n" : "#include \"fused_sinks.hpp\"\n") << "namespace plx { namespace k {\n"
       "struct JitProg {\n  static constexpr bool kStatic = true; static constexpr int kId = -2;\n  static constexpr Shape shape() {\n    Shape s{};\n";
  o << "    s.n_inputs = " << (int)sh.n_inputs << "; s.n_ops = " << (int)sh.n_ops << "; s.n_aggs = " << (int)sh.n_aggs << "; s.pred = " << (int)sh.pred
    << "; s.key = " << (int)sh.key << "; s.n_keys = " << (int)sh.n_keys << ";\n";
  for (int i = 0; i < kMaxKeys; i++) o << "    s.keys[" << i << "] = " << (int)sh.keys[i] << ";\n";
  for (int i = 0; i < sh.n_inputs; i++) o << "    s.in_dtype[" << i << "] = " << (int)sh.in_dtype[i] << "; s.in_nullable[" << i << "] = " << (int)sh.in_nullable[i] << ";\n";
  for (int i = 0; i < sh.n_ops; i++)
    o << "    s.ops[" << i << "] = mkop(" << (int)sh.ops[i].code << ", " << (int)sh.ops[i].dst << ", " << (int)sh.ops[i].a << ", " << (int)sh.ops[i].b << ", " << (int)sh.ops[i].c << ");\n";
  for (int i = 0; i < sh.n_aggs; i++) o << "    s.aggs[" << i << "] = Agg{" << (int)sh.aggs[i].kind << ", " << (int)sh.aggs[i].src << "};\n";
  o << "    return s;\n  }\n};\n";
  switch (sink) {
    case PART_COUNT:
      o << "extern \"C\" __global__ __launch_bounds__(kBlock) void plx_jit_kernel(Shape dsh, Args args, uint32_t log2_parts, unsigned int* hist) {\n"
           "  part_count_body<JitProg>(dsh, args, log2_parts, hist);\n}\n}}\n";
      break;
    case PART_SCATTER:
      o << "extern \"C\" __global__ __launch_bounds__(kBlock) void plx_jit_kernel(Shape dsh, Args args, PartitionPlan pp, const unsigned long long* part_off, "
           "const unsigned long long* wg_prefix, unsigned long long* out) {\n  part_scatter_body<JitProg>(dsh, args, pp, part_off, wg_prefix, out);\n}\n}}\n";
      break;
    case PART_AGG:
      o << "extern \"C\" __global__ __launch_bounds__(kAggBlock) void plx_jit_kernel(Shape dsh, PartitionPlan pp, PartAggParams ap) {\n"
           "  constexpr Shape csh = JitProg::shape(); constexpr RecLayout cl = rec_layout(JitProg::shape());\n  part_agg_body(csh, cl, pp, ap);\n}\n}}\n";
      break;
    case PART2_SCATTER_HASH: case PART2_SCATTER_DIRECT: case PART2_SCATTER_HASH_T2: case PART2_SCATTER_DIRECT_T2:
      o << "extern \"C\" __global__ __launch_bounds__(kP2MaxBlock) void plx_jit_kernel(Shape dsh, Args args, PartPlan2 pp, ScatterParams2 sp) {\n"
           "  part2_scatter_body<JitProg, " << ((sink == PART2_SCATTER_DIRECT || sink == PART2_SCATTER_DIRECT_T2) ? 1 : 0) << ", "
        << ((sink == PART2_SCATTER_HASH_T2 || sink == PART2_SCATTER_DIRECT_T2) ? 2 : 1) << ">(dsh, args, pp, sp);\n}\n}}\n";
      break;
    case PART2_AGG_HASH: case PART2_AGG_DIRECT:
      o << "extern \"C\" __global__ __launch_bounds__(kP2AggBlock) void plx_jit_kernel(PartPlan2 pp, AggParams2 ap) {\n"
           "  constexpr Shape csh = JitProg::shape(); constexpr RecLayout2 cl = rec_layout2(JitProg::shape(), " << (sink == PART2_AGG_DIRECT ? 1 : 0) << "u);\n"
           "  part2_agg_body<Shape, " << (sink == PART2_AGG_DIRECT ? 1 : 0) << ", p2_agg_chunks_in_flight(cl.rec_words)>(csh, cl, pp, ap);\n}\n}}\n";
      break;
    default:
      if (wide_tiles(sink)) {
        o << "extern \"C\" __global__ __launch_bounds__(kBlock) void plx_jit_kernel(Shape dsh, Args args, " << sink_type(sink)
          << "::Params sp) {\n  fused_scan_body<JitProg, " << sink_type(sink) << ", true>(dsh, args, sp);\n}\n}}\n";
        break;
      }
      if (sink == PART3_AGG_PAIRV) {
        o << "extern \"C\" __global__ __launch_bounds__(kP2AggBlock) void plx_jit_kernel(PartPlan2 pp, AggParams2 ap) {\n"
             "  constexpr Shape csh = JitProg::shape(); constexpr RecLayout2 cl = rec_layout2(JitProg::shape(), 0u, " << fused::kPackPairV << "u);\n"
             "  part2_agg_body<Shape, 0, p2_agg_chunks_in_flight(cl.rec_words)>(csh, cl, pp, ap);\n}\n}}\n";
        break;
      }
      if (sink >= PART3_SCATTER_PAIRV && sink < PART3_AGG_PAIRV) {
        const int v = (int)sink - (int)PART3_SCATTER_PAIRV, tiles = 1 + (v & 3), hot = (v >> 2) & 1;
        o << "extern \"C\" __global__ __launch_bounds__(kP2MaxBlock) void plx_jit_kernel(Shape dsh, Args args, PartPlan2 pp, ScatterParams2 sp) {\n"
             "  part3_scatter_body<JitProg, 0, " << tiles << ", " << fused::kPackPairV << ", " << (hot ? "true" : "false") << ">(dsh, args, pp, sp);\n}\n}}\n";
        break;
      }
      if (sink == PART3_AGG_PAIR || sink == PART3_AGG_PAIR_DIRECT) {
        const int mode = sink == PART3_AGG_PAIR_DIRECT ? 1 : 0;
        o << "extern \"C\" __global__ __launch_bounds__(kP2AggBlock) void plx_jit_kernel(PartPlan2 pp, AggParams2 ap) {\n"
             "  constexpr Shape csh = JitProg::shape(); constexpr RecLayout2 cl = rec_layout2(JitProg::shape(), " << mode << "u, " << fused::kPackPair << "u);\n"
             "  part2_agg_body<Shape, " << mode << ", p2_agg_chunks_in_flight(cl.rec_words)>(csh, cl, pp, ap);\n}\n}}\n";
        break;
      }
      if (sink >= PART3_SCATTER_PAIR && sink < PART3_AGG_PAIR) {
        const int v = (int)sink - (int)PART3_SCATTER_PAIR, tiles = 1 + (v & 3), hot = (v >> 2) & 1, mode = v >> 3;
        o << "extern \"C\" __global__ __launch_bounds__(kP2MaxBlock) void plx_jit_kernel(Shape dsh, Args args, PartPlan2 pp, ScatterParams2 sp) {\n"
             "  part3_scatter_body<JitProg, " << mode << ", " << tiles << ", " << fused::kPackPair << ", " << (hot ? "true" : "false") << ">(dsh, args, pp, sp);\n}\n}}\n";
        break;
      }
      if (sink >= PART3_AGG && sink != BALLOT && sink != DIRECT_HITS) {
        const int v = (int)sink - (int)PART3_AGG, mode = v & 1, pack = v >> 1;
        o << "extern \"C\" __global__ __launch_bounds__(kP2AggBlock) void plx_jit_kernel(PartPlan2 pp, AggParams2 ap) {\n"
             "  constexpr Shape csh = JitProg::shape(); constexpr RecLayout2 cl = rec_layout2(JitProg::shape(), " << mode << "u, " << pack << "u);\n"
             "  part2_agg_body<Shape, " << mode << ", p2_agg_chunks_in_flight(cl.rec_words)>(csh, cl, pp, ap);\n}\n}}\n";
        break;
      }
      if (sink >= PART3_SCATTER && sink != BALLOT && sink != DIRECT_HITS) {
        const int v = (int)sink - (int)PART3_SCATTER, mode = v & 1, tiles = 1 + ((v >> 1) & 3), pack = (v >> 3) & 3, hot = v >> 5;
        o << "extern \"C\" __global__ __launch_bounds__(kP2MaxBlock) void plx_jit_kernel(Shape dsh, Args args, PartPlan2 pp, ScatterParams2 sp) {\n"
             "  part3_scatter_body<JitProg, " << mode << ", " << tiles << ", " << pack << ", " << (hot ? "true" : "false") << ">(dsh, args, pp, sp);\n}\n}}\n";
        break;
      }
      o << "extern \"C\" __global__ __launch_bounds__(kBlock) void plx_jit_kernel(Shape dsh, Args args, " << sink_type(sink)
        << "::Params sp) {\n  fused_scan_body<JitProg, " << sink_type(sink) << ">(dsh, args, sp);\n}\n}}\n";
      break;
  }
  return o.str();
}

std::atomic<int64_t> g_min_rows{-2};
bool enabled(int64_t n_rows) {
  int64_t m = g_min_rows.load(std::memory_order_relaxed);
  if (m == -2) {
    const char* off = getenv("PLX_JIT");
    const char* e = getenv("PLX_JIT_MIN_ROWS");
    m = (off && off[0] == '0') ? -1 : (e ? (int64_t)atoll(e) : (int64_t)1 << 22);
    g_min_rows.store(m, std::memory_order_relaxed);
  }
  return m >= 0 && n_rows >= m;
}

std::string cache_dir() {
  const char* off = getenv("PLX_JIT_CACHE");
  if (off && off[0] == '0') return "";
  if (const char* d = getenv("PLX_JIT_CACHE_DIR")) return d;
  const char* home = getenv("HOME");
  return home && *home ? std::string(home) + "/.cache/polars_amd/jit" : std::string("/tmp/polars_amd_jit");
}
std::string headers_fingerprint() {
  static const std::string fp = [] {
    uint64_t h = 0xcbf29ce484222325ull;
    for (const char* f : {"fused.hpp", "fused_device.hpp", "fused_sinks.hpp", "fused_shapes.hpp", "partition_device.hpp", "partition2_device.hpp", "partition3_device.hpp", "dev.hpp", "kconfig.hpp", "temporal.hpp", "decimal.hpp"}) {
      if (FILE* fp2 = fopen((include_dir() + "/" + f).c_str(), "rb")) {
        char buf[65536]; size_t n;
        while ((n = fread(buf, 1, sizeof buf, fp2)) > 0) h = fnv1a(std::string(buf, n), h);
        fclose(fp2);
      }
    }
    char out[32]; snprintf(out, sizeof out, "%016llx", (unsigned long long)h);
    return std::string(out);
  }();
  return fp;
}
std::string cache_path(const std::string& src) {
  const std::string dir = cache_dir();
  if (dir.empty()) return "";
  std::string key = src + "|" + headers_fingerprint();
  for (auto& o : compile_options()) if (o.compare(0, 2, "-I") != 0) key += "|" + o;
  char name[64]; snprintf(name, sizeof name, "/%016llx%016llx.hsaco", (unsigned long long)fnv1a(key), (unsigned long long)fnv1a(key, 0x9e3779b97f4a7c15ull));
  return dir + name;
}
bool load_cached(const std::string& path, std::vector<char>* code) {
  if (path.empty()) return false;
  FILE* f = fopen(path.c_str(), "rb");
  if (!f) return false;
  fseek(f, 0, SEEK_END); const long n = ftell(f); fseek(f, 0, SEEK_SET);
  bool ok = n > 0;
  if (ok) { code->resize((size_t)n); ok = fread(code->data(), 1, (size_t)n, f) == (size_t)n; }
  fclose(f);
  return ok;
}
void store_cached(const std::string& path, const std::vector<char>& code) {
  if (path.empty()) return;
  const std::string dir = path.substr(0, path.rfind('/'));
  std::string acc;
  for (size_t i = 1; i <= dir.size(); i++) if (i == dir.size() || dir[i] == '/') { acc = dir.substr(0, i); (void)mkdir(acc.c_str(), 0755); }
  const std::string tmp = path + ".tmp" + std::to_string((long)getpid());
  if (FILE* f = fopen(tmp.c_str(), "wb")) {
    const bool ok = fwrite(code.data(), 1, code.size(), f) == code.size();
    fclose(f);
    if (!ok || rename(tmp.c_str(), path.c_str()) != 0) (void)remove(tmp.c_str());
  }
}
int g_cache_hits = 0;

Entry compile(const Shape& sh, Sink sink) {
  Entry e;
  const auto t0 = std::chrono::steady_clock::now();
  const std::string src = source_for(sh, sink);
  const std::string cpath = cache_path(src);
  {
    std::vector<char> cached;
    if (load_cached(cpath, &cached) && hipModuleLoadData(&e.mod, cached.data()) == hipSuccess && hipModuleGetFunction(&e.fn, e.mod, kernel_symbol(sh, sink).c_str()) == hipSuccess) {
      g_cache_hits++; g_compiled++;
      if (getenv("PLX_JIT_VERBOSE")) fprintf(stderr, "[plx jit] %s: loaded from %s\n", sink_type(sink), cpath.c_str());
      return e;
    }
    (void)hipGetLastError();
    e = Entry{};
  }
  hiprtcProgram prog = nullptr;
  if (hiprtcCreateProgram(&prog, src.c_str(), "plx_jit.hip", 0, nullptr, nullptr) != HIPRTC_SUCCESS) { e.failed = true; return e; }
  const std::vector<std::string> optv = compile_options();
  std::vector<const char*> opts;
  for (auto& x : optv) opts.push_back(x.c_str());
  const hiprtcResult rc = hiprtcCompileProgram(prog, (int)opts.size(), opts.data());
  if (rc != HIPRTC_SUCCESS) {
    size_t n = 0; hiprtcGetProgramLogSize(prog, &n);
    std::string log(n, 0); if (n) hiprtcGetProgramLog(prog, &log[0]);
    set_last_error("jit: hiprtc compile failed: " + log.substr(0, 2000));
    if (getenv("PLX_JIT_VERBOSE")) fprintf(stderr, "[plx jit] compile failed:\n%s\n", log.c_str());
    hiprtcDestroyProgram(&prog);
    e.failed = true;
    return e;
  }
  size_t cs = 0; hiprtcGetCodeSize(prog, &cs);
  std::vector<char> code(cs);
  hiprtcGetCode(prog, code.data());
  hiprtcDestroyProgram(&prog);
  if (hipModuleLoadData(&e.mod, code.data()) != hipSuccess || hipModuleGetFunction(&e.fn, e.mod, kernel_symbol(sh, sink).c_str()) != hipSuccess) { e.failed = true; return e; }
  const double ms = std::chrono::duration<double, std::milli>(std::chrono::steady_clock::now() - t0).count();
  g_compiled++; g_ms += ms;
  if (getenv("PLX_JIT_VERBOSE")) fprintf(stderr, "[plx jit] %s: %.0f ms, %zu bytes\n", sink_type(sink), ms, cs);
  return e;
}
}

std::string selftest(const Shape& sh, Sink sink) {
  const std::string src = source_for(sh, sink);
  hiprtcProgram prog = nullptr;
  if (hiprtcCreateProgram(&prog, src.c_str(), "plx_jit.hip", 0, nullptr, nullptr) != HIPRTC_SUCCESS) return "hiprtcCreateProgram failed";
  const std::vector<std::string> optv = compile_options();
  std::vector<const char*> opts;
  for (auto& x : optv) opts.push_back(x.c_str());
  const hiprtcResult rc = hiprtcCompileProgram(prog, (int)opts.size(), opts.data());
  std::string log;
  if (rc != HIPRTC_SUCCESS) { size_t n = 0; hiprtcGetProgramLogSize(prog, &n); log.assign(n, 0); if (n) hiprtcGetProgramLog(prog, &log[0]); if (log.empty()) log = "hiprtc error"; }
  else if (const char* dir = getenv("PLX_JIT_DUMP_DIR")) {
    size_t cs = 0; hiprtcGetCodeSize(prog, &cs);
    std::vector<char> code(cs);
    hiprtcGetCode(prog, code.data());
    const std::string base = std::string(dir) + "/" + sink_type(sink) + (wide_tiles(sink) ? "_wide" : "") + "_" + std::to_string((int)sink);
    if (FILE* f = fopen((base + ".hsaco").c_str(), "wb")) { fwrite(code.data(), 1, code.size(), f); fclose(f); }
    if (FILE* f = fopen((base + ".hip").c_str(), "wb")) { fwrite(src.data(), 1, src.size(), f); fclose(f); }
  }
  hiprtcDestroyProgram(&prog);
  return log;
}

const char* program_mode(int static_id, int64_t n_rows) { return static_id >= 0 ? "aot" : (enabled(n_rows) ? "jit" : "generic"); }

void set_min_rows(int64_t min_rows) { g_min_rows.store(min_rows < 0 ? -1 : min_rows, std::memory_order_relaxed); }

void stats(int* compiled, double* compile_ms) {
  std::lock_guard<std::mutex> lk(g_mu);
  if (compiled) *compiled = g_compiled;
  if (compile_ms) *compile_ms = g_ms;
}

static hipFunction_t get_fn(const Shape& sh, Sink sink) {
  std::string key((const char*)&sh, sizeof(Shape));
  key.push_back((char)sink);
  std::lock_guard<std::mutex> lk(g_mu);
  auto it = g_cache.find(key);
  if (it == g_cache.end()) it = g_cache.emplace(key, compile(sh, sink)).first;
  return it->second.failed ? nullptr : it->second.fn;
}

bool ensure(const Shape& sh, Sink kind, int64_t n_rows) { return enabled(n_rows) && get_fn(sh, kind) != nullptr; }

bool launch_raw(const Shape& sh, Sink kind, void** kargs, int grid, int block, size_t lds_bytes) {
  hipFunction_t fn = get_fn(sh, kind);
  if (!fn) return false;
  const hipError_t rc = hipModuleLaunchKernel(fn, (unsigned)grid, 1, 1, (unsigned)block, 1, 1, (unsigned)lds_bytes, stream(), kargs, nullptr);
  if (rc != hipSuccess) { set_last_error(std::string("jit: launch failed: ") + hipGetErrorString(rc)); return false; }
  return true;
}

bool launch(const Shape& sh, const Args& args, Sink sink, const void* params, int grid, size_t lds_bytes) {
  if (!enabled(args.n_rows)) return false;
  Shape shc = sh; Args ac = args;
  void* kargs[] = {(void*)&shc, (void*)&ac, const_cast<void*>(params)};
  return launch_raw(sh, sink, kargs, grid, k::kBlock, lds_bytes);
}

}
}
```

### polars_amd/csrc/jit.hpp

```cpp
#pragma once
#include <cstddef>
#include <cstdint>
#include <string>

#include "fused.hpp"

namespace plx {
namespace jit {

enum Sink { REGAGG = 0, LDSAGG, DENSE, HASH, WIDE, JOIN_BUILD, PROBE_AGG, DIRECT_BUILD, DIRECT_PROBE, BITMAP_BUILD,
            PART_COUNT, PART_SCATTER, PART_AGG,
            PART2_SCATTER_HASH, PART2_SCATTER_DIRECT, PART2_AGG_HASH, PART2_AGG_DIRECT,
            PART2_SCATTER_HASH_T2, PART2_SCATTER_DIRECT_T2,
            PART3_SCATTER, PART3_AGG = PART3_SCATTER + 64,
            BALLOT = PART3_AGG + 8,
            DIRECT_HITS,
            PART3_SCATTER_PAIR, PART3_AGG_PAIR = PART3_SCATTER_PAIR + 16, PART3_AGG_PAIR_DIRECT,
            PART3_SCATTER_PAIRV, PART3_AGG_PAIRV = PART3_SCATTER_PAIRV + 8,
            REGAGG_WIDE, LDSAGG_WIDE,
            kNumSinks };
inline Sink part3_scatter_sink(uint32_t mode, uint32_t tiles, uint32_t pack, bool hot) {
  if (pack == fused::kPackPairV) return (Sink)(PART3_SCATTER_PAIRV + (tiles - 1) + (hot ? 4 : 0));
  if (pack == fused::kPackPair) return (Sink)(PART3_SCATTER_PAIR + (tiles - 1) + (hot ? 4 : 0) + 8 * mode);
  return (Sink)(PART3_SCATTER + mode + 2 * (tiles - 1) + 8 * pack + (hot ? 32 : 0));
}
inline Sink part3_agg_sink(uint32_t mode, uint32_t pack) { return pack == fused::kPackPairV ? PART3_AGG_PAIRV : pack == fused::kPackPair ? (Sink)(PART3_AGG_PAIR + mode) : (Sink)(PART3_AGG + mode + 2 * pack); }

bool launch(const fused::Shape& sh, const fused::Args& args, Sink sink, const void* params, int grid, size_t lds_bytes);
bool ensure(const fused::Shape& sh, Sink kind, int64_t n_rows);
bool launch_raw(const fused::Shape& sh, Sink kind, void** kargs, int grid, int block, size_t lds_bytes);
std::string selftest(const fused::Shape& sh, Sink sink);
const char* program_mode(int static_id, int64_t n_rows);
void set_min_rows(int64_t min_rows);
void stats(int* compiled, double* compile_ms);

}
}
```

### polars_amd/csrc/kernels_fused.hip

```cpp
#include "fused_sinks.hpp"
#include "kernels.hpp"
#include "kernels_fused.hpp"
#include "variance.hpp"
#include "scan.hpp"
#include "jit.hpp"
#include <atomic>
#include <cstring>
#include <vector>

#ifdef PLX_HAVE_Q3_SHAPES
#define PLX_STATIC_JOIN_BUILD_CASES \
  case SHAPE_Q3_BUILD: hipLaunchKernelGGL((fused_scan_kernel<StatProg<SHAPE_Q3_BUILD>, JoinBuildSink>), dim3(grid), dim3(kBlock), 0, stream(), sh, args, t); break; \
  case SHAPE_Q3D_BUILD: hipLaunchKernelGGL((fused_scan_kernel<StatProg<SHAPE_Q3D_BUILD>, JoinBuildSink>), dim3(grid), dim3(kBlock), 0, stream(), sh, args, t); break;
#define PLX_STATIC_PROBE_AGG_CASES \
  case SHAPE_Q3_PROBE: hipLaunchKernelGGL((fused_scan_kernel<StatProg<SHAPE_Q3_PROBE>, ProbeAggSink>), dim3(grid), dim3(kBlock), 0, stream(), sh, args, t); break;
#define PLX_STATIC_REGAGG_EXTRA_CASES \
  case SHAPE_Q3_COUNT: launch_static<SHAPE_Q3_COUNT, RegAggSink>(wide, grid, 0, sh, args, sp); break;
#define PLX_STATIC_DIRECT_BUILD_CASES \
  case SHAPE_Q3_BUILD: hipLaunchKernelGGL((fused_scan_kernel<StatProg<SHAPE_Q3_BUILD>, DirectBuildSink>), dim3(grid), dim3(kBlock), 0, stream(), sh, args, t); break; \
  case SHAPE_Q3D_BUILD: hipLaunchKernelGGL((fused_scan_kernel<StatProg<SHAPE_Q3D_BUILD>, DirectBuildSink>), dim3(grid), dim3(kBlock), 0, stream(), sh, args, t); break;
#define PLX_STATIC_DIRECT_PROBE_CASES \
  case SHAPE_Q3_PROBE: hipLaunchKernelGGL((fused_scan_kernel<StatProg<SHAPE_Q3_PROBE>, DirectProbeAggSink>), dim3(grid), dim3(kBlock), 0, stream(), sh, args, t); break;
#ifdef PLX_HAVE_Q3FULL_SHAPES
#define PLX_STATIC_BITMAP_BUILD_CASES \
  case SHAPE_Q3F_SEMI: hipLaunchKernelGGL((fused_scan_kernel<StatProg<SHAPE_Q3F_SEMI>, BitmapBuildSink>), dim3(grid), dim3(kBlock), 0, stream(), sh, args, t); break;
#define PLX_STATIC_Q3F_JOIN_BUILD_CASES \
  case SHAPE_Q3F_BUILD: hipLaunchKernelGGL((fused_scan_kernel<StatProg<SHAPE_Q3F_BUILD>, JoinBuildSink>), dim3(grid), dim3(kBlock), 0, stream(), sh, args, t); break;
#define PLX_STATIC_Q3F_DIRECT_BUILD_CASES \
  case SHAPE_Q3F_BUILD: hipLaunchKernelGGL((fused_scan_kernel<StatProg<SHAPE_Q3F_BUILD>, DirectBuildSink>), dim3(grid), dim3(kBlock), 0, stream(), sh, args, t); break;
#define PLX_STATIC_Q3F_REGAGG_CASES \
  case SHAPE_Q3F_COUNT: launch_static<SHAPE_Q3F_COUNT, RegAggSink>(wide, grid, 0, sh, args, sp); break;
#else
#define PLX_STATIC_BITMAP_BUILD_CASES
#define PLX_STATIC_Q3F_JOIN_BUILD_CASES
#define PLX_STATIC_Q3F_DIRECT_BUILD_CASES
#define PLX_STATIC_Q3F_REGAGG_CASES
#endif
#else
#define PLX_STATIC_BITMAP_BUILD_CASES
#define PLX_STATIC_Q3F_JOIN_BUILD_CASES
#define PLX_STATIC_Q3F_DIRECT_BUILD_CASES
#define PLX_STATIC_Q3F_REGAGG_CASES
#define PLX_STATIC_DIRECT_BUILD_CASES
#define PLX_STATIC_DIRECT_PROBE_CASES
#define PLX_STATIC_JOIN_BUILD_CASES
#define PLX_STATIC_PROBE_AGG_CASES
#define PLX_STATIC_REGAGG_EXTRA_CASES
#endif

#include <cstdlib>

namespace plx {
namespace k {

static std::string scope_name(const char* aot, const char* other, int static_id) { return static_id >= 0 ? std::string(aot) + "#" + std::to_string(static_id) : std::string(other); }


using namespace dev;
using namespace fused;

__global__ __launch_bounds__(kBlock) void partials_finish_kernel(Shape sh, const unsigned long long* __restrict__ partials, int np, int cells,
                                                                 int cell_stride, unsigned long long* __restrict__ out) {
  __shared__ uint64_t red[kBlock / 64];
  const int cell = blockIdx.x;
  const uint8_t kind = sh.aggs[cell % sh.n_aggs].kind;
  uint64_t x = agg_identity_dev(kind);
  for (int i = threadIdx.x; i < np; i += blockDim.x) x = agg_combine(kind, x, partials[(size_t)i * cell_stride + cell]);
#pragma unroll
  for (int m = 32; m >= 1; m >>= 1) x = agg_combine(kind, x, shfl_xor_u64(x, m));
  if (lane_id() == 0) red[threadIdx.x >> 6] = x;
  __syncthreads();
  if (threadIdx.x == 0) {
    for (int w = 1; w < (int)(blockDim.x >> 6); w++) x = agg_combine(kind, x, red[w]);
    out[cell] = x;
  }
}

static int scan_grid(int64_t n_rows, int blocks_per_cu, const char* knob = nullptr, int tile_rows = kTileRows) {
  if (knob) { const char* e = getenv(knob); const int v = e ? atoi(e) : 0; if (v >= 1 && v <= 32) blocks_per_cu = v; }
  int64_t ntiles = (n_rows + tile_rows - 1) / tile_rows;
  return grid_for(ntiles, kBlock / 64, blocks_per_cu);
}
static_assert(!trust_nullable<StatProg<SHAPE_Q1>, LdsAggSink>() && !trust_nullable<StatProg<SHAPE_CFG2>, RegAggSink>() && !trust_nullable<StatProg<SHAPE_CFG2_NULLX>, RegAggSink>(),
// ... 28 lines not shown
template <int ID, class Sink>
static void launch_static(bool wide, int grid, size_t lds, const Shape& sh, const Args& args, const typename Sink::Params& sp) {
  if constexpr (wide_tiles_form<StatProg<ID>, Sink>()) {
    if (wide) { hipLaunchKernelGGL((fused_scan_wide_kernel<StatProg<ID>, Sink>), dim3(grid), dim3(kBlock), lds, stream(), sh, args, sp); return; }
  }
  PLX_REQUIRE(!wide, PLX_ERR_INVALID, "fused scan: no wide-tile kernel for this shape");
  PLX_LAUNCH_SCAN(StatProg<ID>, Sink, grid, lds, sh, args, sp);
}

void fused_regagg(const Shape& sh, const Args& args, int static_id, uint64_t* out_host) {
  const bool wide = wide_tiles_choice(sh, args, static_id >= 0 || jit::program_mode(static_id, args.n_rows)[0] == 'j', wide_tiles_knob());
  g_last_tile_rows.store(wide ? kWideTileRows : kTileRows, std::memory_order_relaxed);
  const int grid = scan_grid(args.n_rows, 5, "PLX_BPC_REGAGG", wide ? kWideTileRows : kTileRows);
  Buf partials = dev_alloc(sizeof(uint64_t) * (size_t)(grid + 1) * kMaxAggs);
  unsigned long long* pp = partials->as<unsigned long long>();
  RegAggSink::Params sp{pp};
  {
    ProfileScope ps(scope_name("fused_scan_regagg_static", "fused_scan_regagg_generic", static_id).c_str(), algo_bytes(sh, args), (uint64_t)args.n_rows);
    switch (static_id) {
      case SHAPE_CFG2: launch_static<SHAPE_CFG2, RegAggSink>(wide, grid, 0, sh, args, sp); break;
      case SHAPE_CFG2_NULLX: launch_static<SHAPE_CFG2_NULLX, RegAggSink>(wide, grid, 0, sh, args, sp); break;
      case SHAPE_CFG1: launch_static<SHAPE_CFG1, RegAggSink>(wide, grid, 0, sh, args, sp); break;
      PLX_STATIC_REGAGG_EXTRA_CASES
      PLX_STATIC_Q3F_REGAGG_CASES
      default:
        if (!jit::launch(sh, args, wide ? jit::REGAGG_WIDE : jit::REGAGG, &sp, grid, 0)) {
          g_last_tile_rows.store(kTileRows, std::memory_order_relaxed);
          const DynLaunch d = dyn_launch(sh, args, 0); PLX_LAUNCH_SCAN(DynProg, RegAggSink, grid, d.lds, sh, d.args, sp);
        }
        break;
    }
    PLX_HIP(hipGetLastError());
  }
  unsigned long long* fin = pp + (size_t)grid * kMaxAggs;
  hipLaunchKernelGGL(partials_finish_kernel, dim3(sh.n_aggs), dim3(kBlock), 0, stream(), sh, pp, grid, (int)sh.n_aggs, (int)kMaxAggs, fin);
  PLX_HIP(hipGetLastError());
  d2h_sync(out_host, fin, (size_t)sh.n_aggs * 8);
}

void fused_ballots(const Shape& sh, const Args& args, const BallotOut& out, int static_id) {
  if (args.n_rows == 0) return;
  ProfileScope ps(scope_name("fused_scan_ballots_static", jit::program_mode(-1, args.n_rows)[0] == 'j' ? "fused_scan_ballots[jit]" : "fused_scan_ballots[generic]", static_id).c_str(),
                  algo_bytes(sh, args), (uint64_t)args.n_rows);
  const int grid = scan_grid(args.n_rows, 5, "PLX_BPC_BALLOTS");
  if (!jit::launch(sh, args, jit::BALLOT, &out, grid, 0)) { const DynLaunch d = dyn_launch(sh, args, 0); hipLaunchKernelGGL((fused_scan_kernel<DynProg, BallotSink>), dim3(grid), dim3(kBlock), d.lds, stream(), sh, d.args, out); }
  PLX_HIP(hipGetLastError());
}

void fused_direct_hits(const Shape& sh, const Args& args, const DirectJoinTable& t, const BallotOut& out, int static_id) {
  if (args.n_rows == 0) return;
  ProfileScope ps(scope_name("fused_scan_direct_hits_static", "fused_scan_direct_hits", static_id).c_str(), algo_bytes(sh, args), (uint64_t)args.n_rows);
  const int grid = scan_grid(args.n_rows, 8, "PLX_BPC_DIRECT_HITS");
  DirectHits p{t, out};
  switch (static_id) {
#ifdef PLX_HAVE_Q3_PROBE_SCATTER
    case SHAPE_Q3_PROBE_SCATTER: hipLaunchKernelGGL((fused_scan_kernel<StatProg<SHAPE_Q3_PROBE_SCATTER>, DirectHitsSink>), dim3(grid), dim3(kBlock), 0, stream(), sh, args, p); break;
#endif
    default: if (!jit::launch(sh, args, jit::DIRECT_HITS, &p, grid, 0)) { const DynLaunch d = dyn_launch(sh, args, 0); hipLaunchKernelGGL((fused_scan_kernel<DynProg, DirectHitsSink>), dim3(grid), dim3(kBlock), d.lds, stream(), sh, d.args, p); } break;
  }
  PLX_HIP(hipGetLastError());
}
__global__ __launch_bounds__(kBlock) void direct_slot_rows_kernel(DirectJoinTable t, int64_t n_used, unsigned int* __restrict__ slot_row) {
  for (int64_t o = (int64_t)blockIdx.x * blockDim.x + threadIdx.x; o < n_used; o += (int64_t)gridDim.x * blockDim.x) {
    if ((unsigned int)(o % kOrdChunk) >= t.chunk_used[o / kOrdChunk]) continue;
    const unsigned long long idx = t.ord_key[o] - (unsigned long long)t.kmin;
    slot_row[direct_slot(t, idx, t.bits[idx >> 6])] = t.ord_row[o];
  }
}
void direct_slot_rows(const DirectJoinTable& t, int64_t n_used, uint32_t* slot_row) {
  if (n_used == 0) return;
  ProfileScope ps("direct_slot_rows", (uint64_t)n_used * 28, (uint64_t)n_used);
  hipLaunchKernelGGL(direct_slot_rows_kernel, dim3(grid_for(n_used, kBlock * 4)), dim3(kBlock), 0, stream(), t, n_used, (unsigned int*)slot_row);
  PLX_HIP(hipGetLastError());
}

int lds_agg_copies(int n_groups, int n_aggs) {
  const size_t budget = 60 * 1024;
  int c = 16;
  while (c > 1 && (size_t)n_groups * n_aggs * c * 8 > budget) c >>= 1;
  if ((size_t)n_groups * n_aggs * c * 8 > budget) return 0;
  return c;
}

void fused_lds_agg(const Shape& sh, const Args& args, int n_groups, int static_id, uint64_t* out_dev , unsigned int* oob) {
  const int copies = lds_agg_copies(n_groups, sh.n_aggs);
  PLX_REQUIRE(copies > 0, PLX_ERR_INVALID, "fused_lds_agg: group table does not fit LDS");
  const int cells = n_groups * sh.n_aggs;
  const size_t lds = (size_t)cells * copies * 8;
  const bool wide = wide_tiles_choice(sh, args, static_id >= 0 || jit::program_mode(static_id, args.n_rows)[0] == 'j', wide_tiles_knob());
  g_last_tile_rows.store(wide ? kWideTileRows : kTileRows, std::memory_order_relaxed);
  const int grid = scan_grid(args.n_rows, 5, "PLX_BPC_LDSAGG", wide ? kWideTileRows : kTileRows);
  const bool use_partials = n_groups <= 64;
  Buf partials;
  LdsAggSink::Params sp{};
  sp.n_groups = n_groups; sp.copies = copies; sp.oob = oob;
  if (use_partials) { partials = dev_alloc(sizeof(uint64_t) * (size_t)grid * cells); sp.partials = partials->as<unsigned long long>(); }
  else { init_agg_cells(out_dev, n_groups, sh); sp.global_acc = (unsigned long long*)out_dev; }
  {
    ProfileScope ps(scope_name("fused_scan_ldsagg_static", "fused_scan_ldsagg_generic", static_id).c_str(), algo_bytes(sh, args), (uint64_t)args.n_rows);
    switch (static_id) {
      case SHAPE_Q1: launch_static<SHAPE_Q1, LdsAggSink>(wide, grid, lds, sh, args, sp); break;
      case SHAPE_Q1_ENCODED: launch_static<SHAPE_Q1_ENCODED, LdsAggSink>(wide, grid, lds, sh, args, sp); break;
      case SHAPE_Q1_ENCODED_PRICE: launch_static<SHAPE_Q1_ENCODED_PRICE, LdsAggSink>(wide, grid, lds, sh, args, sp); break;
      default:
        if (!jit::launch(sh, args, wide ? jit::LDSAGG_WIDE : jit::LDSAGG, &sp, grid, lds)) {
          g_last_tile_rows.store(kTileRows, std::memory_order_relaxed);
          const DynLaunch d = dyn_launch(sh, args, lds); PLX_LAUNCH_SCAN(DynProg, LdsAggSink, grid, d.lds, sh, d.args, sp);
        }
        break;
    }
    PLX_HIP(hipGetLastError());
  }
  if (use_partials) {
    hipLaunchKernelGGL(partials_finish_kernel, dim3(cells), dim3(kBlock), 0, stream(), sh, sp.partials, grid, cells, cells, (unsigned long long*)out_dev);
    PLX_HIP(hipGetLastError());
  }
}

__global__ __launch_bounds__(kBlock) void fill_u64_kernel(unsigned long long* p, int64_t n, unsigned long long v) {
  for (int64_t i = (int64_t)blockIdx.x * blockDim.x + threadIdx.x; i < n; i += (int64_t)gridDim.x * blockDim.x) p[i] = v;
}
__global__ __launch_bounds__(kBlock) void init_acc_kernel(unsigned long long* acc, int64_t n_slots, Shape sh) {
  const int64_t total = n_slots * sh.n_aggs;
  for (int64_t i = (int64_t)blockIdx.x * blockDim.x + threadIdx.x; i < total; i += (int64_t)gridDim.x * blockDim.x)
    acc[i] = agg_identity_dev(sh.aggs[i % sh.n_aggs].kind);
}
void fill_u64(uint64_t* p, int64_t n, uint64_t v) {
  if (n == 0) return;
  hipLaunchKernelGGL(fill_u64_kernel, dim3(grid_for(n, kBlock * 4)), dim3(kBlock), 0, stream(), (unsigned long long*)p, n, (unsigned long long)v);
  PLX_HIP(hipGetLastError());
}
void init_agg_cells(uint64_t* acc, int64_t n_slots, const Shape& sh) {
  if (n_slots == 0) return;
  hipLaunchKernelGGL(init_acc_kernel, dim3(grid_for(n_slots * sh.n_aggs, kBlock * 4)), dim3(kBlock), 0, stream(), (unsigned long long*)acc, n_slots, sh);
  PLX_HIP(hipGetLastError());
}

void fused_dense_agg(const Shape& sh, const Args& args, const DenseTable& t, int static_id) {
  if (args.n_rows == 0) return;
  ProfileScope ps("fused_scan_denseagg", algo_bytes(sh, args), (uint64_t)args.n_rows);
  const int grid = scan_grid(args.n_rows, 8);
  switch (static_id) {
    case SHAPE_GB_SUM_CNT_I64: hipLaunchKernelGGL((fused_scan_kernel<StatProg<SHAPE_GB_SUM_CNT_I64>, DenseAggSink>), dim3(grid), dim3(kBlock), 0, stream(), sh, args, t); break;
    case SHAPE_GB_SUM_MEAN_U32_F64: hipLaunchKernelGGL((fused_scan_kernel<StatProg<SHAPE_GB_SUM_MEAN_U32_F64>, DenseAggSink>), dim3(grid), dim3(kBlock), 0, stream(), sh, args, t); break;
    default: if (!jit::launch(sh, args, jit::DENSE, &t, grid, 0)) { const DynLaunch d = dyn_launch(sh, args, 0); hipLaunchKernelGGL((fused_scan_kernel<DynProg, DenseAggSink>), dim3(grid), dim3(kBlock), d.lds, stream(), sh, d.args, t); } break;
  }
  PLX_HIP(hipGetLastError());
}

void fused_hash_agg(const Shape& sh, const Args& args, const HashTable& t, int static_id) {
  if (args.n_rows == 0) return;
  ProfileScope ps("fused_scan_hashagg", algo_bytes(sh, args), (uint64_t)args.n_rows);
  const int grid = scan_grid(args.n_rows, 8);
  switch (static_id) {
    case SHAPE_GB_SUM_CNT_I64: hipLaunchKernelGGL((fused_scan_kernel<StatProg<SHAPE_GB_SUM_CNT_I64>, HashAggSink>), dim3(grid), dim3(kBlock), 0, stream(), sh, args, t); break;
    case SHAPE_GB_SUM_MEAN_U32_F64: hipLaunchKernelGGL((fused_scan_kernel<StatProg<SHAPE_GB_SUM_MEAN_U32_F64>, HashAggSink>), dim3(grid), dim3(kBlock), 0, stream(), sh, args, t); break;
    default: if (!jit::launch(sh, args, jit::HASH, &t, grid, 0)) { const DynLaunch d = dyn_launch(sh, args, 0); hipLaunchKernelGGL((fused_scan_kernel<DynProg, HashAggSink>), dim3(grid), dim3(kBlock), d.lds, stream(), sh, d.args, t); } break;
  }
  PLX_HIP(hipGetLastError());
}



constexpr int kCompactItems = 8;
template <class Occ, class Emit>
__device__ __forceinline__ void compact_slots(int64_t n_slots, unsigned long long* counter, Occ occ, Emit emit) {
  __shared__ uint32_t wave_tot[kBlock / 64];
  __shared__ unsigned long long chunk_base;
  const int lane = lane_id(), wave = threadIdx.x >> 6;
  const int64_t chunk = (int64_t)kBlock * kCompactItems;
  const int64_t nchunks = (n_slots + chunk - 1) / chunk;
  for (int64_t c = blockIdx.x; c < nchunks; c += gridDim.x) {
    const int64_t s0 = c * chunk + threadIdx.x;
    uint32_t bits = 0;
#pragma unroll
    for (int j = 0; j < kCompactItems; j++) { const int64_t s = s0 + (int64_t)j * kBlock; if (s < n_slots && occ(s)) bits |= 1u << j; }
    const uint32_t cnt = (uint32_t)__popc(bits);
    uint32_t incl = cnt;
#pragma unroll
    for (int d = 1; d < 64; d <<= 1) { const uint32_t o = __shfl_up(incl, d, 64); if (lane >= d) incl += o; }
    if (lane == 63) wave_tot[wave] = incl;
    __syncthreads();
    uint32_t wave_off = 0, total = 0;
#pragma unroll
    for (int w = 0; w < kBlock / 64; w++) { if (w < wave) wave_off += wave_tot[w]; total += wave_tot[w]; }
    if (threadIdx.x == 0 && total) chunk_base = atomicAdd(counter, (unsigned long long)total);
    __syncthreads();
    if (total) {
      uint64_t o = chunk_base + wave_off + (incl - cnt);
#pragma unroll
      for (int j = 0; j < kCompactItems; j++) if ((bits >> j) & 1) { emit(s0 + (int64_t)j * kBlock, o); o++; }
    }
    __syncthreads();
  }
}
// ... 559 lines not shown
```

### polars_amd/csrc/kernels_fused.hpp

```cpp
#pragma once
#include <string>
#include <vector>

#include "core.hpp"
#include "fused.hpp"

namespace plx {
namespace k {

void fused_regagg(const fused::Shape& sh, const fused::Args& args, int static_id, uint64_t* out_host);
int lds_agg_copies(int n_groups, int n_aggs);
void fused_lds_agg(const fused::Shape& sh, const fused::Args& args, int n_groups, int static_id, uint64_t* out_dev, unsigned int* oob = nullptr );

bool wide_tiles_choice(const fused::Shape& sh, const fused::Args& args, bool compiled, bool knob_on);
int last_scan_tile_rows();

void fused_dense_agg(const fused::Shape& sh, const fused::Args& args, const fused::DenseTable& t, int static_id);
void fused_hash_agg(const fused::Shape& sh, const fused::Args& args, const fused::HashTable& t, int static_id);
void fused_wide_agg(const fused::Shape& sh, const fused::Args& args, const fused::WideTable& t);
int64_t wide_compact(const fused::WideTable& t, int n_keys, int n_aggs, int64_t out_stride, uint64_t* out_words, uint8_t* out_kvalid, uint64_t* out_acc);
void fused_join_build(const fused::Shape& sh, const fused::Args& args, const fused::JoinAggTable& t, int static_id);
void fused_probe_agg(const fused::Shape& sh, const fused::Args& args, const fused::JoinAggTable& t, int static_id);
int64_t join_agg_compact(const fused::JoinAggTable& t, int n_aggs, int len_idx, uint64_t* out_keys, uint32_t* out_rows, uint64_t* out_acc);
void canonicalise_chains(const fused::JoinAggTable& t, const fused::RepCols& rc, unsigned int max_chain, unsigned int* flags);
int64_t rows_agg_compact(const uint64_t* acc, int64_t n_rows, int n_aggs, int len_idx, uint32_t* out_rows, uint64_t* out_acc);
int64_t chains_agg_compact(const fused::JoinAggTable& t, const fused::Shape& sh, const uint64_t* acc, int len_idx, Buf* out_rows, Buf* out_acc);
int64_t scan_waves(int64_t n_rows);
void fused_ballots(const fused::Shape& sh, const fused::Args& args, const fused::BallotOut& out, int static_id);
void fused_bitmap_build(const fused::Shape& sh, const fused::Args& args, const fused::BitmapBuild& t, int static_id);
void fused_direct_build(const fused::Shape& sh, const fused::Args& args, const fused::DirectJoinTable& t, int static_id);
void fused_direct_probe_agg(const fused::Shape& sh, const fused::Args& args, const fused::DirectJoinTable& t, int static_id);
void fused_direct_hits(const fused::Shape& sh, const fused::Args& args, const fused::DirectJoinTable& t, const fused::BallotOut& out, int static_id);
void direct_slot_rows(const fused::DirectJoinTable& t, int64_t n_used, uint32_t* slot_row);
uint64_t direct_rank(const fused::DirectJoinTable& t, uint32_t* rank_out, int64_t n_used, uint64_t* n_pairs_dev, uint64_t* pairs_out);
int64_t direct_agg_compact(const fused::DirectJoinTable& t, int64_t n_used, int n_aggs, int len_idx, uint64_t* out_keys, uint32_t* out_rows, uint64_t* out_acc);
void fill_u64(uint64_t* p, int64_t n, uint64_t v);
void init_agg_cells(uint64_t* acc, int64_t n_slots, const fused::Shape& sh);
int64_t table_compact(const uint64_t* keys, const uint64_t* acc, int64_t n_slots, int64_t cap, int n_aggs, int occ_agg, uint64_t* out_keys,
                      uint8_t* out_key_valid, uint64_t* out_acc);

void finalize_aggs(const uint64_t* acc, int n_aggs, int64_t G, const fused::FinalSpec& sp, void* out, uint64_t* out_valid);
bool partition_plan(const fused::Shape& sh, double est_groups, bool any_nullable, fused::PartitionPlan* out);
int64_t partitioned_agg(const fused::Shape& sh, const fused::Args& args, const fused::PartitionPlan& pp, int static_id, Buf* out_keys, Buf* out_kvalid,
                        Buf* out_acc, std::string* desc);
struct SrcRange { bool known = false; int64_t mn = 0, mx = 0; bool check = false;  };
bool partition_plan2(const fused::Shape& sh, double est_groups, int packed_bits, int len_idx, int64_t n_rows, int n_hot, fused::PartPlan2* out,
                     const SrcRange* src_ranges = nullptr , const SrcRange* key_range = nullptr );
void select_hot_keys(const fused::HashTable& t, int n_aggs, int len_idx, uint64_t threshold, std::vector<uint64_t>* out, uint64_t* hot_rows = nullptr);
int64_t partitioned_agg2(const fused::Shape& sh, const fused::Args& args, const fused::PartPlan2& pp, int static_id, const std::vector<uint64_t>& hot_keys, Buf* out_keys,
                         Buf* out_kvalid, Buf* out_acc, std::string* desc, int64_t* key_range_out = nullptr, int64_t* wide_stride_out = nullptr);
void touch_filter_set(const int64_t* keys, const uint64_t* validity, int64_t n, unsigned int log2_bits, uint64_t* filter);
bool partitioned_probe_hits(const fused::Shape& sh, const fused::Args& args, const fused::DirectJoinTable& dt, uint64_t n_build, int static_id, ColumnPtr* hits, std::string* desc);
bool partitioned_hash_probe_hits(const fused::Shape& sh, const fused::Args& args, const fused::JoinAggTable& ht, uint64_t n_build, int static_id, ColumnPtr* hits, std::string* desc);
struct JoinCells { Buf key, row; };
bool partitioned_join_build(const fused::Shape& sh, const fused::Args& args, int static_id, const fused::JoinAggTable& t, JoinCells* cells, std::string* desc);
int64_t cells_agg_compact(const JoinCells& cells, const uint64_t* acc, int64_t n_cells, int n_aggs, int len_idx, uint64_t* out_keys, uint32_t* out_rows, uint64_t* out_acc);
double sample_sortedness(const ColumnPtr& c);
bool sample_minmax(const ColumnPtr& c, int64_t* mn, int64_t* mx, int blocks = 64);
void finalize_batch(const uint64_t* acc, int n_aggs, int64_t G, const fused::FinBatch& b);
void decode_key(const uint64_t* packed, const uint8_t* kvalid, int64_t G, const fused::KeyDecode& kd, void* out, uint64_t* out_valid);

}
}
```

Measured before the change: 398.5 billion rows/s.

## Share LDS aggregation cells between count, integer sum and derived float sums

Adds a cell plan for the LDS group-by aggregation. When the value bounds are known, the row count and a bounded non-negative integer sum are packed into one 64-bit LDS word, with the count stored above a computed shift. Float sums and means that are exact conversions of that integer sum are then derived from the same cell instead of being accumulated separately. This cuts LDS atomics and footprint per row for encoded Q1 shapes, which can also allow more table copies. The cost is new planning logic, static and JIT kernel variants, and correctness that depends on trusted range metadata and overflow bounds.

```diff
diff --git a/include/polars_amd.h b/include/polars_amd.h
--- a/include/polars_amd.h
+++ b/include/polars_amd.h
@@ -319,6 +319,11 @@
 const char* plx_last_plan_description(void);
 const char* plx_last_plan_encodings(void);
 int32_t plx_last_scan_tile_rows(void);
+int32_t plx_last_lds_cells(void);
+void plx_set_shared_cells(int32_t on);
+int32_t plx_cell_plan(int32_t static_shape_id, int32_t n_inputs, const int32_t* dtypes, const int32_t* nullable, int32_t n_ops, const uint8_t* ops, int32_t n_aggs, const uint8_t* aggs,
+                      const uint8_t* known, const int64_t* lo, const int64_t* hi, uint64_t wg_rows, uint64_t n_rows, int32_t* out);
+uint64_t plx_lds_wg_rows(int64_t n_rows, int32_t grid, int32_t wide);
 int32_t plx_wide_tiles_choice(int32_t compiled, int32_t knob_on, int64_t n_rows, int32_t n_inputs, const int32_t* dtypes, const int32_t* nullable, const uint64_t* values,
                               const uint64_t* validity);
 
diff --git a/polars_amd/_ffi.py b/polars_amd/_ffi.py
--- a/polars_amd/_ffi.py
+++ b/polars_amd/_ffi.py
@@ -240,6 +240,11 @@
     "plx_last_plan_description": (C.c_char_p, []),
     "plx_last_plan_encodings": (C.c_char_p, []),
     "plx_last_scan_tile_rows": (C.c_int32, []),
+    "plx_last_lds_cells": (C.c_int32, []),
+    "plx_set_shared_cells": (None, [C.c_int32]),
+    "plx_cell_plan": (C.c_int32, [C.c_int32, C.c_int32, C.POINTER(C.c_int32), C.POINTER(C.c_int32), C.c_int32, C.POINTER(C.c_uint8), C.c_int32, C.POINTER(C.c_uint8),
+                                  C.POINTER(C.c_uint8), C.POINTER(C.c_int64), C.POINTER(C.c_int64), C.c_uint64, C.c_uint64, C.POINTER(C.c_int32)]),
+    "plx_lds_wg_rows": (C.c_uint64, [C.c_int64, C.c_int32, C.c_int32]),
     "plx_wide_tiles_choice": (C.c_int32, [C.c_int32, C.c_int32, C.c_int64, C.c_int32, C.POINTER(C.c_int32), C.POINTER(C.c_int32), C.POINTER(C.c_uint64), C.POINTER(C.c_uint64)]),
     "plx_profile_enable": (C.c_int, [C.c_int]),
     "plx_profile_fetch": (C.c_int, [C.POINTER(ProfileRecord), C.c_int32, _i32p]),
@@ -310,6 +315,29 @@
     return int(lib().plx_last_scan_tile_rows())
 
 
+def last_lds_cells() -> int:
+    return int(lib().plx_last_lds_cells())
+
+
+def set_shared_cells(on: bool) -> None:
+    lib().plx_set_shared_cells(int(bool(on)))
+
+
+def cell_plan(facts, wg_rows, n_rows, static_shape_id=-1, dtypes=(), nullable=(), ops=(), aggs=()):
+    n_aggs = len(facts)
+    ni, no = len(dtypes), len(ops)
+    out = (C.c_int32 * (2 + 2 * 16))()
+    flat_ops = [int(x) for op in ops for x in op]
+    flat_aggs = [int(x) for a in aggs for x in a]
+    r = lib().plx_cell_plan(int(static_shape_id), ni, (C.c_int32 * max(ni, 1))(*[int(d) for d in dtypes]), (C.c_int32 * max(ni, 1))(*[int(x) for x in nullable]),
+                            no, (C.c_uint8 * max(len(flat_ops), 1))(*flat_ops), len(aggs), (C.c_uint8 * max(len(flat_aggs), 1))(*flat_aggs),
+                            (C.c_uint8 * 16)(*[int(f[0]) for f in facts]), (C.c_int64 * 16)(*[int(f[1]) for f in facts]), (C.c_int64 * 16)(*[int(f[2]) for f in facts]),
+                            int(wg_rows), int(n_rows), out)
+    if r < 0:
+        raise ValueError("plx_cell_plan: bad arguments")
+    return int(out[0]), int(out[1]), [int(out[2 + k]) for k in range(r)], [int(out[2 + r + k]) for k in range(r)]
+
+
 def wide_tiles_choice(compiled, knob_on, n_rows, dtypes, nullable, values, validity) -> int:
     n = len(dtypes)
     return int(lib().plx_wide_tiles_choice(int(bool(compiled)), int(bool(knob_on)), int(n_rows), n, (C.c_int32 * n)(*[int(d) for d in dtypes]),
diff --git a/polars_amd/csrc/abi.cpp b/polars_amd/csrc/abi.cpp
--- a/polars_amd/csrc/abi.cpp
+++ b/polars_amd/csrc/abi.cpp
@@ -1221,6 +1221,32 @@
 const char* plx_last_plan_description(void) { return t_plan_desc.c_str(); }
 const char* plx_last_plan_encodings(void) { return t_plan_encoded.c_str(); }
 int32_t plx_last_scan_tile_rows(void) { return k::last_scan_tile_rows(); }
+int32_t plx_last_lds_cells(void) { return k::last_lds_cells(); }
+void plx_set_shared_cells(int32_t on) { k::set_shared_cells(on != 0); }
+uint64_t plx_lds_wg_rows(int64_t n_rows, int32_t grid, int32_t wide) { return (n_rows < 0 || grid < 1) ? 0 : k::lds_agg_wg_rows_of(n_rows, grid, wide != 0); }
+int32_t plx_cell_plan(int32_t static_shape_id, int32_t n_inputs, const int32_t* dtypes, const int32_t* nullable, int32_t n_ops, const uint8_t* ops, int32_t n_aggs, const uint8_t* aggs,
+                      const uint8_t* known, const int64_t* lo, const int64_t* hi, uint64_t wg_rows, uint64_t n_rows, int32_t* out) {
+  if (!known || !lo || !hi || !out) return -1;
+  fused::Shape sh{};
+  if (static_shape_id >= 0) {
+    if (static_shape_id >= fused::kNumStaticShapes) return -1;
+    sh = fused::static_shape(static_shape_id);
+  } else {
+    if (n_inputs < 0 || n_inputs > fused::kMaxInputs || n_ops < 0 || n_ops > fused::kMaxOps || n_aggs < 0 || n_aggs > fused::kMaxAggs) return -1;
+    if ((n_inputs && (!dtypes || !nullable)) || (n_ops && !ops) || (n_aggs && !aggs)) return -1;
+    sh.n_inputs = (uint8_t)n_inputs; sh.n_ops = (uint8_t)n_ops; sh.n_aggs = (uint8_t)n_aggs; sh.pred = fused::kNone; sh.key = fused::kNone;
+    for (int i = 0; i < n_inputs; i++) { sh.in_dtype[i] = (uint8_t)dtypes[i]; sh.in_nullable[i] = (uint8_t)(nullable[i] != 0); }
+    for (int i = 0; i < n_ops; i++) sh.ops[i] = fused::Op{ops[5 * i], ops[5 * i + 1], ops[5 * i + 2], ops[5 * i + 3], ops[5 * i + 4], {0, 0, 0}};
+    for (int i = 0; i < n_aggs; i++) sh.aggs[i] = fused::Agg{aggs[2 * i], aggs[2 * i + 1]};
+  }
+  fused::AggFacts f{};
+  f.wg_rows = wg_rows; f.n_rows = n_rows;
+  for (int k = 0; k < sh.n_aggs; k++) { f.known[k] = known[k]; f.lo[k] = lo[k]; f.hi[k] = hi[k]; }
+  const fused::CellPlan p = fused::plan_cells(sh, f);
+  out[0] = p.n_cells; out[1] = p.shift;
+  for (int k = 0; k < sh.n_aggs; k++) { out[2 + k] = p.cell[k]; out[2 + sh.n_aggs + k] = p.from[k] == fused::kNone ? -1 : (int)p.from[k]; }
+  return sh.n_aggs;
+}
 int32_t plx_wide_tiles_choice(int32_t compiled, int32_t knob_on, int64_t n_rows, int32_t n_inputs, const int32_t* dtypes, const int32_t* nullable, const uint64_t* values,
                               const uint64_t* validity) {
   if (n_inputs < 0 || n_inputs > fused::kMaxInputs || (n_inputs && (!dtypes || !nullable || !values || !validity))) return -1;
@@ -1348,6 +1374,11 @@
   for (auto& j : jobs) {
     const std::string log = jit::selftest(j.first, j.second);
     if (!log.empty()) fail(PLX_ERR_INVALID, "jit selftest failed: " + log.substr(0, 4000));
+    if (j.second != jit::LDSAGG && j.second != jit::LDSAGG_WIDE) continue;
+    const uint32_t code = fused::full_cell_plan_code(j.first);
+    if (fused::cell_plan_is_identity(fused::cell_plan_from_code(j.first, code), j.first)) continue;
+    const std::string log2 = jit::selftest(j.first, j.second == jit::LDSAGG ? jit::LDSCELL : jit::LDSCELL_WIDE, code);
+    if (!log2.empty()) fail(PLX_ERR_INVALID, "jit selftest failed: " + log2.substr(0, 4000));
   }
   PLX_CATCH
 }
diff --git a/polars_amd/csrc/engine.cpp b/polars_amd/csrc/engine.cpp
--- a/polars_amd/csrc/engine.cpp
+++ b/polars_amd/csrc/engine.cpp
@@ -1314,11 +1314,47 @@
   check_oob_flag(oob);
   q.res.key_valid = nullptr;
 }
+bool input_value_bounds(const GroupByRun& q, int i, int64_t* lo, int64_t* hi) {
+  if (i < 0 || i >= (int)q.c.input_cols.size() || q.args.in[i].validity) return false;
+  const ColumnPtr& col = q.c.cols[q.c.input_cols[i]];
+  const std::shared_ptr<EncodedShadow> s = std::atomic_load(&col->shadow);
+  const bool codes = s && s->kind == EncodedShadow::kAffine && s->codes && q.args.in[i].values == s->codes->ptr;
+  if (!codes && q.args.in[i].values != col->data()) {
+    const char* p = (const char*)q.args.in[i].values; const char* b = (const char*)col->data();
+    if (!b || p < b || p >= b + (size_t)col->len * dtype_width(col->dtype) || q.sh.in_dtype[i] != col->dtype) return false;
+  }
+  switch (q.sh.in_dtype[i]) {
+    case PLX_U8: *lo = 0; *hi = 255; return true;
+    case PLX_U16: *lo = 0; *hi = 65535; return true;
+    case PLX_U32: *lo = 0; *hi = 0xffffffffll; return true;
+    case PLX_I8: *lo = -128; *hi = 127; return true;
+    case PLX_I16: *lo = -32768; *hi = 32767; return true;
+    case PLX_I32: *lo = INT32_MIN; *hi = INT32_MAX; return true;
+    case PLX_I64: case PLX_U64:
+      if (codes || col->range_state != 1 || !col->range_trusted || col->range_assumed) return false;
+      if (q.sh.in_dtype[i] == PLX_U64 && col->range_min < 0) return false;
+      *lo = col->range_min; *hi = col->range_max; return true;
+    default: return false;
+  }
+}
+CellPlan shared_cells_plan(const GroupByRun& q) {
+  AggFacts f{};
+  f.n_rows = (uint64_t)q.args.n_rows; f.wg_rows = k::lds_agg_wg_rows(q.args.n_rows);
+  for (int k = 0; k < q.sh.n_aggs; k++) {
+    if (q.sh.aggs[k].kind != AGG_SUM_I) continue;
+    const int in = affine_source_input(q.sh, q.sh.aggs[k].src);
+    int64_t lo = 0, hi = 0;
+    if (in < 0 || !input_value_bounds(q, in, &lo, &hi) || !affine_source_interval(q.sh, q.args, q.sh.aggs[k].src, &lo, &hi)) continue;
+    f.known[k] = 1; f.lo[k] = lo; f.hi[k] = hi;
+  }
+  return plan_cells(q.sh, f);
+}
 void lds_table(GroupByRun& q) {
   const int G = 1 << q.kp.total_bits;
   Buf cells = dev_alloc(sizeof(uint64_t) * (size_t)G * q.sh.n_aggs);
   Buf oob = untrusted_key_bounds(q.c) ? dev_alloc_zero(8) : nullptr;
-  k::fused_lds_agg(q.sh, q.args, G, q.static_id, cells->as<uint64_t>(), oob ? oob->as<unsigned int>() : nullptr);
+  const CellPlan cell_plan = shared_cells_plan(q);
+  k::fused_lds_agg(q.sh, q.args, G, q.static_id, cells->as<uint64_t>(), oob ? oob->as<unsigned int>() : nullptr, &cell_plan);
   q.desc += scan_tag(q.static_id, q.args.n_rows) + "lds_table(G=" + std::to_string(G) + ",copies=" + std::to_string(k::lds_agg_copies(G, q.sh.n_aggs)) + ")";
   finish_table(q, cells, G, oob);
 }
diff --git a/polars_amd/csrc/fused_cells.hpp b/polars_amd/csrc/fused_cells.hpp
--- /dev/null
+++ b/polars_amd/csrc/fused_cells.hpp
@@ -0,0 +1,148 @@
+#pragma once
+#include "fused.hpp"
+
+namespace plx {
+namespace fused {
+
+struct AggFacts {
+  uint8_t known[kMaxAggs];
+  int64_t lo[kMaxAggs], hi[kMaxAggs];
+  uint64_t wg_rows;
+  uint64_t n_rows;
+};
+struct CellPlan {
+  uint8_t n_cells;
+  uint8_t packed;
+  uint8_t packed_len;
+  uint8_t shift;
+  uint8_t cell[kMaxAggs];
+  uint8_t from[kMaxAggs];
+  uint8_t owner[kMaxAggs];
+};
+constexpr uint32_t kIdentityCells = 0xffffu;
+PLX_HD constexpr uint32_t cell_plan_code(uint8_t packed, uint8_t packed_len, uint32_t derived) { return (uint32_t)packed | ((uint32_t)packed_len << 8) | (derived << 16); }
+
+PLX_HD constexpr int bits_u64(uint64_t x) { int b = 0; while (x) { b++; x >>= 1; } return b; }
+
+PLX_HD constexpr int affine_source_input(const Shape& sh, uint8_t slot) {
+  int input = -1;
+  for (int pc = 0; pc < sh.n_ops; pc++) {
+    const Op op = sh.ops[pc];
+    if (op.code == OP_NOP || op.dst != slot) continue;
+    if (op.code == OP_LOAD) {
+      if (input >= 0 || op.a >= sh.n_inputs || sh.in_nullable[op.a]) return -1;
+      const uint8_t dt = sh.in_dtype[op.a];
+      if (dt < 1 || dt > 8) return -1;
+      input = op.a;
+      continue;
+    }
+    if (input < 0 || (op.code != OP_MUL_I && op.code != OP_ADD_I) || op.a != slot || op.b == slot) return -1;
+    int def = -1;
+    for (int q = 0; q < pc; q++) if (sh.ops[q].code != OP_NOP && sh.ops[q].dst == op.b) def = q;
+    if (def < 0 || sh.ops[def].code != OP_CONST) return -1;
+  }
+  return input;
+}
+PLX_HD constexpr uint8_t i2f_sum_source(const Shape& sh, int k) {
+  if (k >= sh.n_aggs || sh.aggs[k].kind != AGG_SUM_F) return kNone;
+  const uint8_t d = sh.aggs[k].src;
+  int def = -1;
+  for (int pc = 0; pc < sh.n_ops; pc++) if (sh.ops[pc].code != OP_NOP && sh.ops[pc].dst == d) def = pc;
+  if (def < 0 || sh.ops[def].code != OP_I2F || sh.ops[def].a == d) return kNone;
+  const uint8_t s = sh.ops[def].a;
+  for (int pc = def + 1; pc < sh.n_ops; pc++) if (sh.ops[pc].code != OP_NOP && sh.ops[pc].dst == s) return kNone;
+  if (affine_source_input(sh, s) < 0) return kNone;
+  for (int j = 0; j < sh.n_aggs; j++) if (sh.aggs[j].kind == AGG_SUM_I && sh.aggs[j].src == s) return (uint8_t)j;
+  return kNone;
+}
+
+PLX_HD constexpr CellPlan cell_plan_from_code(const Shape& sh, uint32_t code) {
+  CellPlan p{};
+  p.packed = kNone; p.packed_len = kNone; p.shift = 0;
+  for (int k = 0; k < kMaxAggs; k++) { p.cell[k] = 0; p.from[k] = kNone; p.owner[k] = 0; }
+  if ((code & 0xffffu) != kIdentityCells) {
+    p.packed = (uint8_t)(code & 0xffu); p.packed_len = (uint8_t)((code >> 8) & 0xffu);
+    p.from[p.packed_len] = p.packed;
+  }
+  for (int k = 0; k < sh.n_aggs; k++) if ((code >> (16 + k)) & 1u) p.from[k] = i2f_sum_source(sh, k);
+  uint8_t n = 0;
+  for (int k = 0; k < sh.n_aggs; k++) if (p.from[k] == kNone) { p.cell[k] = n; p.owner[n] = (uint8_t)k; n++; }
+  for (int k = 0; k < sh.n_aggs; k++) if (p.from[k] != kNone) p.cell[k] = p.cell[p.from[k]];
+  p.n_cells = n;
+  return p;
+}
+PLX_HD constexpr uint32_t cell_plan_code(const CellPlan& p, const Shape& sh) {
+  uint32_t derived = 0;
+  for (int k = 0; k < sh.n_aggs; k++) if (p.from[k] != kNone && k != p.packed_len) derived |= 1u << k;
+  return p.packed == kNone ? (kIdentityCells | (derived << 16)) : cell_plan_code(p.packed, p.packed_len, derived);
+}
+PLX_HD constexpr bool cell_plan_is_identity(const CellPlan& p, const Shape& sh) { return p.n_cells == sh.n_aggs; }
+
+PLX_HD constexpr bool exact_f64_sum(int64_t lo, int64_t hi, uint64_t n_rows) {
+  const uint64_t a = lo < 0 ? (uint64_t)0 - (uint64_t)lo : (uint64_t)lo, b = hi < 0 ? (uint64_t)0 - (uint64_t)hi : (uint64_t)hi;
+  const uint64_t m = a > b ? a : b;
+  if (m == 0 || n_rows == 0) return true;
+  const uint64_t lim = 1ull << 53;
+  return m < lim && n_rows <= (lim - 1) / m;
+}
+PLX_HD constexpr int packed_shift(uint64_t wg_rows, int64_t hi) {
+  if (hi < 0 || wg_rows == 0) return -1;
+  const uint64_t h = (uint64_t)hi;
+  if (h != 0 && wg_rows > ~0ull / h) return -1;
+  const int s = bits_u64(wg_rows * h);
+  return bits_u64(wg_rows) + s <= 64 ? s : -1;
+}
+
+PLX_HD constexpr uint64_t packed_row(uint32_t shift, uint64_t v) { return (1ull << shift) + v; }
+PLX_HD constexpr uint64_t packed_count(uint64_t word, uint32_t shift) { return word >> shift; }
+PLX_HD constexpr uint64_t packed_sum(uint64_t word, uint32_t shift) { return word & ((1ull << shift) - 1ull); }
+
+PLX_HD constexpr CellPlan plan_cells(const Shape& sh, const AggFacts& f) {
+  uint8_t packed = kNone, packed_len = kNone;
+  int shift = 0;
+  int len = -1, n_len = 0;
+  for (int k = 0; k < sh.n_aggs; k++) if (sh.aggs[k].kind == AGG_LEN) { if (len < 0) len = k; n_len++; }
+  if (n_len == 1) {
+    for (int k = 0; k < sh.n_aggs && packed == kNone; k++) {
+      if (sh.aggs[k].kind != AGG_SUM_I || !f.known[k] || f.lo[k] < 0 || affine_source_input(sh, sh.aggs[k].src) < 0) continue;
+      const int s = packed_shift(f.wg_rows, f.hi[k]);
+      if (s < 0) continue;
+      packed = (uint8_t)k; packed_len = (uint8_t)len; shift = s;
+    }
+  }
+  uint32_t derived = 0;
+  for (int k = 0; k < sh.n_aggs; k++) {
+    const uint8_t j = i2f_sum_source(sh, k);
+    if (j == kNone || j != packed || !exact_f64_sum(f.lo[j], f.hi[j], f.n_rows)) continue;
+    derived |= 1u << k;
+  }
+  CellPlan p = cell_plan_from_code(sh, packed == kNone ? (kIdentityCells | (derived << 16)) : cell_plan_code(packed, packed_len, derived));
+  p.shift = (uint8_t)shift;
+  return p;
+}
+PLX_HD constexpr uint32_t full_cell_plan_code(const Shape& sh) {
+  AggFacts f{};
+  for (int k = 0; k < kMaxAggs; k++) { f.known[k] = 1; f.lo[k] = 0; f.hi[k] = 1; }
+  f.wg_rows = 1; f.n_rows = 1;
+  return cell_plan_code(plan_cells(sh, f), sh);
+}
+
+inline bool affine_source_interval(const Shape& sh, const Args& a, uint8_t slot, int64_t* lo, int64_t* hi) {
+  for (int pc = 0; pc < sh.n_ops; pc++) {
+    const Op op = sh.ops[pc];
+    if (op.code == OP_NOP || op.dst != slot || op.code == OP_LOAD) continue;
+    int def = -1;
+    for (int q = 0; q < pc; q++) if (sh.ops[q].code != OP_NOP && sh.ops[q].dst == op.b) def = q;
+    if (def < 0) return false;
+    const int64_t c = (int64_t)a.imm[def];
+    int64_t x = 0, y = 0;
+    if (op.code == OP_MUL_I) { if (__builtin_mul_overflow(*lo, c, &x) || __builtin_mul_overflow(*hi, c, &y)) return false; }
+    else if (op.code == OP_ADD_I) { if (__builtin_add_overflow(*lo, c, &x) || __builtin_add_overflow(*hi, c, &y)) return false; }
+    else return false;
+    *lo = x < y ? x : y; *hi = x < y ? y : x;
+  }
+  return true;
+}
+
+}
+}
diff --git a/polars_amd/csrc/fused_sinks.hpp b/polars_amd/csrc/fused_sinks.hpp
--- a/polars_amd/csrc/fused_sinks.hpp
+++ b/polars_amd/csrc/fused_sinks.hpp
@@ -1,6 +1,7 @@
 #pragma once
 #include <type_traits>
 
+#include "fused_cells.hpp"
 #include "fused_device.hpp"
 
 namespace plx {
@@ -99,6 +100,79 @@
     }
   }
 };
+
+template <class P, uint32_t CODE>
+struct LdsCellSink {
+  static constexpr CellPlan kPlan = cell_plan_from_code(P::shape(), CODE);
+  static constexpr int NC = kPlan.n_cells;
+  struct Params {
+    unsigned long long* partials;
+    unsigned long long* global_acc;
+    int n_groups;
+    int copies;
+    unsigned int* oob;
+    unsigned int shift;
+  };
+  template <class S> __device__ __forceinline__ void init(const S& sh, const Params& p) {
+    extern __shared__ unsigned long long lds_tbl[];
+    const int cells = p.n_groups * NC;
+    for (int i = threadIdx.x; i < cells * p.copies; i += blockDim.x) lds_tbl[i] = agg_identity_dev(sh.aggs[kPlan.owner[(i / p.copies) % NC]].kind);
+    __syncthreads();
+  }
+  template <class S, class RF> __device__ __forceinline__ void consume(const S& sh, const RF& rf, const bool pass[kRows], int64_t row0, const Params& p) {
+    extern __shared__ unsigned long long lds_tbl[];
+    constexpr CellPlan pl = kPlan;
+    const int copy = lane_id() & (p.copies - 1);
+#pragma unroll
+    for (int r = 0; r < kRows; r++) {
+      if (!pass[r]) continue;
+      const uint64_t gid64 = rf.get(r, sh.key);
+      if (gid64 >= (uint64_t)p.n_groups) { if (p.oob) *p.oob = 1u; continue; }
+      const uint32_t gid = (uint32_t)gid64;
+      unsigned long long* cells = lds_tbl + (size_t)gid * NC * p.copies + copy;
+#pragma unroll
+      for (int k = 0; k < kMaxAggs; k++) {
+        if (k < sh.n_aggs) {
+          if (pl.from[k] != kNone) continue;
+          const Agg ag = sh.aggs[k];
+          uint64_t v = rf.get(r, ag.src);
+          if (k == pl.packed) { atomicAdd(cells + pl.cell[k] * p.copies, (unsigned long long)packed_row(p.shift, v)); continue; }
+          bool valid = (rf.getv(ag.src) >> r) & 1;
+          if ((ag.kind == AGG_SUM_F || ag.kind == AGG_SUM_I || ag.kind == AGG_COUNT) && !valid) continue;
+          uint64_t x = agg_row_value(ag.kind, v, true, valid, (uint64_t)(row0 + r));
+          lds_atomic_agg(ag.kind, cells + pl.cell[k] * p.copies, x);
+        }
+      }
+    }
+  }
+  template <class S> __device__ __forceinline__ void finish(const S& sh, const Params& p) {
+    extern __shared__ unsigned long long lds_tbl[];
+    constexpr CellPlan pl = kPlan;
+    __syncthreads();
+    const int held = p.n_groups * NC;
+    for (int i = threadIdx.x; i < held; i += blockDim.x) {
+      const uint8_t kind = sh.aggs[pl.owner[i % NC]].kind;
+      uint64_t x = lds_tbl[(size_t)i * p.copies];
+      for (int c = 1; c < p.copies; c++) x = agg_combine(kind, x, lds_tbl[(size_t)i * p.copies + c]);
+      lds_tbl[(size_t)i * p.copies] = x;
+    }
+    __syncthreads();
+    const int cells = p.n_groups * sh.n_aggs;
+    for (int i = threadIdx.x; i < cells; i += blockDim.x) {
+      const int g = i / sh.n_aggs, k = i % sh.n_aggs;
+      const uint8_t kind = sh.aggs[k].kind;
+      uint64_t x = lds_tbl[((size_t)g * NC + pl.cell[k]) * p.copies];
+      if (pl.packed != kNone && pl.cell[k] == pl.cell[pl.packed]) {
+        x = k == pl.packed_len ? packed_count(x, p.shift) : packed_sum(x, p.shift);
+        if (k != pl.packed && k != pl.packed_len) x = as_u((double)(long long)x);
+      } else if (pl.from[k] != kNone) x = as_u((double)(long long)x);
+      if (p.global_acc) { if (x != agg_identity_dev(kind) || kind == AGG_SUM_F) atomic_agg(kind, p.global_acc + i, x); }
+      else p.partials[(size_t)blockIdx.x * cells + i] = x;
+    }
+  }
+};
+template <class Sink> struct is_lds_table_sink : std::is_same<Sink, LdsAggSink> {};
+template <class P, uint32_t CODE> struct is_lds_table_sink<LdsCellSink<P, CODE>> : std::true_type {};
 
 struct DenseAggSink {
   using Params = DenseTable;
@@ -503,7 +577,7 @@
 }
 template <class P, class Sink>
 __host__ __device__ constexpr bool trust_nullable() {
-  if constexpr (P::kStatic && (std::is_same<Sink, LdsAggSink>::value || std::is_same<Sink, RegAggSink>::value)) return narrow_rows(P::shape());
+  if constexpr (P::kStatic && (is_lds_table_sink<Sink>::value || std::is_same<Sink, RegAggSink>::value)) return narrow_rows(P::shape());
   else return false;
 }
 template <class P, class Sink>
diff --git a/polars_amd/csrc/jit.cpp b/polars_amd/csrc/jit.cpp
--- a/polars_amd/csrc/jit.cpp
+++ b/polars_amd/csrc/jit.cpp
@@ -31,12 +31,14 @@
 int g_compiled = 0;
 double g_ms = 0;
 
-bool wide_tiles(Sink s) { return s == REGAGG_WIDE || s == LDSAGG_WIDE; }
+bool wide_tiles(Sink s) { return s == REGAGG_WIDE || s == LDSAGG_WIDE || s == LDSCELL_WIDE; }
+bool shared_cells(Sink s) { return s == LDSCELL || s == LDSCELL_WIDE; }
 const char* sink_type(Sink s) {
   static const char* n[] = {"RegAggSink", "LdsAggSink", "DenseAggSink", "HashAggSink", "WideAggSink", "JoinBuildSink", "ProbeAggSink", "DirectBuildSink", "DirectProbeAggSink", "BitmapBuildSink",
                             "part_count", "part_scatter", "part_agg", "part2_scatter_hash", "part2_scatter_direct", "part2_agg_hash", "part2_agg_direct", "part2_scatter_hash_t2", "part2_scatter_direct_t2"};
   if (s == REGAGG_WIDE) return "RegAggSink";
   if (s == LDSAGG_WIDE) return "LdsAggSink";
+  if (shared_cells(s)) return "LdsCellSink";
   if (s == PART3_AGG_PAIRV) return "part3_agg";
   if (s >= PART3_SCATTER_PAIRV && s < PART3_AGG_PAIRV) return "part3_scatter";
   if (s == PART3_AGG_PAIR || s == PART3_AGG_PAIR_DIRECT) return "part3_agg";
@@ -79,19 +81,20 @@
 
 uint64_t fnv1a(const std::string& s, uint64_t h = 0xcbf29ce484222325ull) { for (unsigned char c : s) { h ^= c; h *= 0x100000001b3ull; } return h; }
 
-std::string kernel_symbol(const Shape& sh, Sink sink) {
+std::string kernel_symbol(const Shape& sh, Sink sink, uint32_t cell_code) {
   std::string key((const char*)&sh, sizeof(Shape));
   key.push_back((char)sink);
+  if (shared_cells(sink)) key.append((const char*)&cell_code, sizeof cell_code);
   char out[96];
   snprintf(out, sizeof out, "plx_jit_%s_%d_%08x", sink_type(sink), (int)sink, (unsigned)(fnv1a(key) & 0xffffffffu));
   return out;
 }
 
-std::string source_for(const Shape& sh, Sink sink) {
+std::string source_for(const Shape& sh, Sink sink, uint32_t cell_code) {
   std::ostringstream o;
-  const std::string sym = kernel_symbol(sh, sink);
+  const std::string sym = kernel_symbol(sh, sink, cell_code);
   o << "#define plx_jit_kernel " << sym << "\n";
-  o << ((sink == BALLOT || sink == DIRECT_HITS || wide_tiles(sink)) ? "#include \"fused_sinks.hpp\"\n" : sink >= PART3_SCATTER ? "#include \"partition3_device.hpp\"\n" : sink >= PART2_SCATTER_HASH ? "#include \"partition2_device.hpp\"\n" : sink >= PART_COUNT ? "#include \"partition_device.hpp\"\n" : "#include \"fused_sinks.hpp\"\n") << "namespace plx { namespace k {\n"
+  o << ((sink == BALLOT || sink == DIRECT_HITS || wide_tiles(sink) || shared_cells(sink)) ? "#include \"fused_sinks.hpp\"\n" : sink >= PART3_SCATTER ? "#include \"partition3_device.hpp\"\n" : sink >= PART2_SCATTER_HASH ? "#include \"partition2_device.hpp\"\n" : sink >= PART_COUNT ? "#include \"partition_device.hpp\"\n" : "#include \"fused_sinks.hpp\"\n") << "namespace plx { namespace k {\n"
        "struct JitProg {\n  static constexpr bool kStatic = true; static constexpr int kId = -2;\n  static constexpr Shape shape() {\n    Shape s{};\n";
   o << "    s.n_inputs = " << (int)sh.n_inputs << "; s.n_ops = " << (int)sh.n_ops << "; s.n_aggs = " << (int)sh.n_aggs << "; s.pred = " << (int)sh.pred
     << "; s.key = " << (int)sh.key << "; s.n_keys = " << (int)sh.n_keys << ";\n";
@@ -125,6 +128,11 @@
            "  part2_agg_body<Shape, " << (sink == PART2_AGG_DIRECT ? 1 : 0) << ", p2_agg_chunks_in_flight(cl.rec_words)>(csh, cl, pp, ap);\n}\n}}\n";
       break;
     default:
+      if (shared_cells(sink)) {
+        o << "extern \"C\" __global__ __launch_bounds__(kBlock) void plx_jit_kernel(Shape dsh, Args args, LdsCellSink<JitProg, " << cell_code << "u>::Params sp) {\n"
+             "  fused_scan_body<JitProg, LdsCellSink<JitProg, " << cell_code << "u>" << (wide_tiles(sink) ? ", true" : "") << ">(dsh, args, sp);\n}\n}}\n";
+        break;
+      }
       if (wide_tiles(sink)) {
         o << "extern \"C\" __global__ __launch_bounds__(kBlock) void plx_jit_kernel(Shape dsh, Args args, " << sink_type(sink)
           << "::Params sp) {\n  fused_scan_body<JitProg, " << sink_type(sink) << ", true>(dsh, args, sp);\n}\n}}\n";
@@ -197,7 +205,7 @@
 std::string headers_fingerprint() {
   static const std::string fp = [] {
     uint64_t h = 0xcbf29ce484222325ull;
-    for (const char* f : {"fused.hpp", "fused_device.hpp", "fused_sinks.hpp", "fused_shapes.hpp", "partition_device.hpp", "partition2_device.hpp", "partition3_device.hpp", "dev.hpp", "kconfig.hpp", "temporal.hpp", "decimal.hpp"}) {
+    for (const char* f : {"fused.hpp", "fused_cells.hpp", "fused_device.hpp", "fused_sinks.hpp", "fused_shapes.hpp", "partition_device.hpp", "partition2_device.hpp", "partition3_device.hpp", "dev.hpp", "kconfig.hpp", "temporal.hpp", "decimal.hpp"}) {
       if (FILE* fp2 = fopen((include_dir() + "/" + f).c_str(), "rb")) {
         char buf[65536]; size_t n;
         while ((n = fread(buf, 1, sizeof buf, fp2)) > 0) h = fnv1a(std::string(buf, n), h);
@@ -241,14 +249,14 @@
 }
 int g_cache_hits = 0;
 
-Entry compile(const Shape& sh, Sink sink) {
+Entry compile(const Shape& sh, Sink sink, uint32_t cell_code) {
   Entry e;
   const auto t0 = std::chrono::steady_clock::now();
-  const std::string src = source_for(sh, sink);
+  const std::string src = source_for(sh, sink, cell_code);
   const std::string cpath = cache_path(src);
   {
     std::vector<char> cached;
-    if (load_cached(cpath, &cached) && hipModuleLoadData(&e.mod, cached.data()) == hipSuccess && hipModuleGetFunction(&e.fn, e.mod, kernel_symbol(sh, sink).c_str()) == hipSuccess) {
+    if (load_cached(cpath, &cached) && hipModuleLoadData(&e.mod, cached.data()) == hipSuccess && hipModuleGetFunction(&e.fn, e.mod, kernel_symbol(sh, sink, cell_code).c_str()) == hipSuccess) {
       g_cache_hits++; g_compiled++;
       if (getenv("PLX_JIT_VERBOSE")) fprintf(stderr, "[plx jit] %s: loaded from %s\n", sink_type(sink), cpath.c_str());
       return e;
@@ -275,7 +283,7 @@
   std::vector<char> code(cs);
   hiprtcGetCode(prog, code.data());
   hiprtcDestroyProgram(&prog);
-  if (hipModuleLoadData(&e.mod, code.data()) != hipSuccess || hipModuleGetFunction(&e.fn, e.mod, kernel_symbol(sh, sink).c_str()) != hipSuccess) { e.failed = true; return e; }
+  if (hipModuleLoadData(&e.mod, code.data()) != hipSuccess || hipModuleGetFunction(&e.fn, e.mod, kernel_symbol(sh, sink, cell_code).c_str()) != hipSuccess) { e.failed = true; return e; }
   const double ms = std::chrono::duration<double, std::milli>(std::chrono::steady_clock::now() - t0).count();
   g_compiled++; g_ms += ms;
   if (getenv("PLX_JIT_VERBOSE")) fprintf(stderr, "[plx jit] %s: %.0f ms, %zu bytes\n", sink_type(sink), ms, cs);
@@ -283,8 +291,8 @@
 }
 }
 
-std::string selftest(const Shape& sh, Sink sink) {
-  const std::string src = source_for(sh, sink);
+std::string selftest(const Shape& sh, Sink sink, uint32_t cell_code) {
+  const std::string src = source_for(sh, sink, cell_code);
   hiprtcProgram prog = nullptr;
   if (hiprtcCreateProgram(&prog, src.c_str(), "plx_jit.hip", 0, nullptr, nullptr) != HIPRTC_SUCCESS) return "hiprtcCreateProgram failed";
   const std::vector<std::string> optv = compile_options();
@@ -297,7 +305,8 @@
     size_t cs = 0; hiprtcGetCodeSize(prog, &cs);
     std::vector<char> code(cs);
     hiprtcGetCode(prog, code.data());
-    const std::string base = std::string(dir) + "/" + sink_type(sink) + (wide_tiles(sink) ? "_wide" : "") + "_" + std::to_string((int)sink);
+    if (shared_cells(sink)) (void)mkdir((std::string(dir) + "/shared_cells").c_str(), 0755);
+    const std::string base = std::string(dir) + (shared_cells(sink) ? "/shared_cells/" : "/") + sink_type(sink) + (wide_tiles(sink) ? "_wide" : "") + "_" + std::to_string((int)sink);
     if (FILE* f = fopen((base + ".hsaco").c_str(), "wb")) { fwrite(code.data(), 1, code.size(), f); fclose(f); }
     if (FILE* f = fopen((base + ".hip").c_str(), "wb")) { fwrite(src.data(), 1, src.size(), f); fclose(f); }
   }
@@ -315,12 +324,13 @@
   if (compile_ms) *compile_ms = g_ms;
 }
 
-static hipFunction_t get_fn(const Shape& sh, Sink sink) {
+static hipFunction_t get_fn(const Shape& sh, Sink sink, uint32_t cell_code = 0) {
   std::string key((const char*)&sh, sizeof(Shape));
   key.push_back((char)sink);
+  if (shared_cells(sink)) key.append((const char*)&cell_code, sizeof cell_code);
   std::lock_guard<std::mutex> lk(g_mu);
   auto it = g_cache.find(key);
-  if (it == g_cache.end()) it = g_cache.emplace(key, compile(sh, sink)).first;
+  if (it == g_cache.end()) it = g_cache.emplace(key, compile(sh, sink, cell_code)).first;
   return it->second.failed ? nullptr : it->second.fn;
 }
 
@@ -334,12 +344,17 @@
   return true;
 }
 
-bool launch(const Shape& sh, const Args& args, Sink sink, const void* params, int grid, size_t lds_bytes) {
+bool launch(const Shape& sh, const Args& args, Sink sink, const void* params, int grid, size_t lds_bytes, uint32_t cell_code) {
   if (!enabled(args.n_rows)) return false;
   Shape shc = sh; Args ac = args;
   void* kargs[] = {(void*)&shc, (void*)&ac, const_cast<void*>(params)};
-  return launch_raw(sh, sink, kargs, grid, k::kBlock, lds_bytes);
-}
-
-}
-}
+  if (!shared_cells(sink)) return launch_raw(sh, sink, kargs, grid, k::kBlock, lds_bytes);
+  hipFunction_t fn = get_fn(sh, sink, cell_code);
+  if (!fn) return false;
+  const hipError_t rc = hipModuleLaunchKernel(fn, (unsigned)grid, 1, 1, (unsigned)k::kBlock, 1, 1, (unsigned)lds_bytes, stream(), kargs, nullptr);
+  if (rc != hipSuccess) { set_last_error(std::string("jit: launch failed: ") + hipGetErrorString(rc)); return false; }
+  return true;
+}
+
+}
+}
diff --git a/polars_amd/csrc/jit.hpp b/polars_amd/csrc/jit.hpp
--- a/polars_amd/csrc/jit.hpp
+++ b/polars_amd/csrc/jit.hpp
@@ -18,6 +18,7 @@
             PART3_SCATTER_PAIR, PART3_AGG_PAIR = PART3_SCATTER_PAIR + 16, PART3_AGG_PAIR_DIRECT,
             PART3_SCATTER_PAIRV, PART3_AGG_PAIRV = PART3_SCATTER_PAIRV + 8,
             REGAGG_WIDE, LDSAGG_WIDE,
+            LDSCELL, LDSCELL_WIDE,
             kNumSinks };
 inline Sink part3_scatter_sink(uint32_t mode, uint32_t tiles, uint32_t pack, bool hot) {
   if (pack == fused::kPackPairV) return (Sink)(PART3_SCATTER_PAIRV + (tiles - 1) + (hot ? 4 : 0));
@@ -26,10 +27,10 @@
 }
 inline Sink part3_agg_sink(uint32_t mode, uint32_t pack) { return pack == fused::kPackPairV ? PART3_AGG_PAIRV : pack == fused::kPackPair ? (Sink)(PART3_AGG_PAIR + mode) : (Sink)(PART3_AGG + mode + 2 * pack); }
 
-bool launch(const fused::Shape& sh, const fused::Args& args, Sink sink, const void* params, int grid, size_t lds_bytes);
+bool launch(const fused::Shape& sh, const fused::Args& args, Sink sink, const void* params, int grid, size_t lds_bytes, uint32_t cell_code = 0 );
 bool ensure(const fused::Shape& sh, Sink kind, int64_t n_rows);
 bool launch_raw(const fused::Shape& sh, Sink kind, void** kargs, int grid, int block, size_t lds_bytes);
-std::string selftest(const fused::Shape& sh, Sink sink);
+std::string selftest(const fused::Shape& sh, Sink sink, uint32_t cell_code = 0);
 const char* program_mode(int static_id, int64_t n_rows);
 void set_min_rows(int64_t min_rows);
 void stats(int* compiled, double* compile_ms);
diff --git a/polars_amd/csrc/kernels_fused.hip b/polars_amd/csrc/kernels_fused.hip
--- a/polars_amd/csrc/kernels_fused.hip
+++ b/polars_amd/csrc/kernels_fused.hip
@@ -1,4 +1,5 @@
 #include "fused_sinks.hpp"
+#include "fused_cells.hpp"
 #include "kernels.hpp"
 #include "kernels_fused.hpp"
 #include "variance.hpp"
@@ -193,12 +194,51 @@
   return c;
 }
 
-void fused_lds_agg(const Shape& sh, const Args& args, int n_groups, int static_id, uint64_t* out_dev , unsigned int* oob) {
-  const int copies = lds_agg_copies(n_groups, sh.n_aggs);
+static std::atomic<int> g_shared_cells{-1};
+static bool shared_cells_knob() {
+  int v = g_shared_cells.load(std::memory_order_relaxed);
+  if (v < 0) { const char* e = getenv("PLX_SHARED_CELLS"); v = (e && e[0] == '0') ? 0 : 1; g_shared_cells.store(v, std::memory_order_relaxed); }
+  return v != 0;
+}
+void set_shared_cells(bool on) { g_shared_cells.store(on ? 1 : 0, std::memory_order_relaxed); }
+static std::atomic<int> g_last_lds_cells{0};
+int last_lds_cells() { return g_last_lds_cells.load(std::memory_order_relaxed); }
+uint64_t lds_agg_wg_rows_of(int64_t n_rows, int grid, bool wide) {
+  const int64_t wpw = kBlock / 64, nwaves = (int64_t)grid * wpw;
+  const int64_t nwide = wide ? n_rows / kWideTileRows : 0;
+  const int64_t rest = (n_rows - nwide * kWideTileRows + kTileRows - 1) / kTileRows;
+  const int64_t per_wave = (nwide + nwaves - 1) / nwaves * kWideTileRows + (rest + nwaves - 1) / nwaves * kTileRows;
+  const int64_t r = wpw * per_wave;
+  return (uint64_t)(r < n_rows ? r : n_rows);
+}
+uint64_t lds_agg_wg_rows(int64_t n_rows) {
+  const uint64_t a = lds_agg_wg_rows_of(n_rows, scan_grid(n_rows, 5, "PLX_BPC_LDSAGG", kWideTileRows), true);
+  const uint64_t b = lds_agg_wg_rows_of(n_rows, scan_grid(n_rows, 5, "PLX_BPC_LDSAGG", kTileRows), false);
+  return a > b ? a : b;
+}
+template <int ID> using SharedCellSink = LdsCellSink<StatProg<ID>, full_cell_plan_code(static_shape(ID))>;
+static_assert(SharedCellSink<SHAPE_Q1_ENCODED>::NC == 5 && SharedCellSink<SHAPE_Q1_ENCODED_PRICE>::NC == 5, "encoded Q1: count, sum and mean of the quantity share one cell");
+static_assert(wide_tiles_form<StatProg<SHAPE_Q1_ENCODED_PRICE>, SharedCellSink<SHAPE_Q1_ENCODED_PRICE>>() && wide_tiles_form<StatProg<SHAPE_Q1_ENCODED>, SharedCellSink<SHAPE_Q1_ENCODED>>(),
+              "the shared-cell kernels have the wide-tile form of the kernels they stand in for");
+static uint32_t static_shared_code(int static_id) {
+  switch (static_id) {
+    case SHAPE_Q1_ENCODED: return full_cell_plan_code(static_shape(SHAPE_Q1_ENCODED));
+    case SHAPE_Q1_ENCODED_PRICE: return full_cell_plan_code(static_shape(SHAPE_Q1_ENCODED_PRICE));
+    default: return kIdentityCells;
+  }
+}
+
+void fused_lds_agg(const Shape& sh, const Args& args, int n_groups, int static_id, uint64_t* out_dev , unsigned int* oob, const CellPlan* cell_plan) {
+  const bool compiled = static_id >= 0 || jit::program_mode(static_id, args.n_rows)[0] == 'j';
+  CellPlan plan = cell_plan_from_code(sh, kIdentityCells);
+  if (cell_plan && compiled && shared_cells_knob() && !cell_plan_is_identity(*cell_plan, sh) && (static_id < 0 || cell_plan_code(*cell_plan, sh) == static_shared_code(static_id))) plan = *cell_plan;
+  bool shared = !cell_plan_is_identity(plan, sh);
+  const uint32_t code = cell_plan_code(plan, sh);
+  int copies = lds_agg_copies(n_groups, plan.n_cells);
   PLX_REQUIRE(copies > 0, PLX_ERR_INVALID, "fused_lds_agg: group table does not fit LDS");
   const int cells = n_groups * sh.n_aggs;
-  const size_t lds = (size_t)cells * copies * 8;
-  const bool wide = wide_tiles_choice(sh, args, static_id >= 0 || jit::program_mode(static_id, args.n_rows)[0] == 'j', wide_tiles_knob());
+  size_t lds = (size_t)n_groups * plan.n_cells * copies * 8;
+  const bool wide = wide_tiles_choice(sh, args, compiled, wide_tiles_knob());
   g_last_tile_rows.store(wide ? kWideTileRows : kTileRows, std::memory_order_relaxed);
   const int grid = scan_grid(args.n_rows, 5, "PLX_BPC_LDSAGG", wide ? kWideTileRows : kTileRows);
   const bool use_partials = n_groups <= 64;
@@ -207,21 +247,37 @@
   sp.n_groups = n_groups; sp.copies = copies; sp.oob = oob;
   if (use_partials) { partials = dev_alloc(sizeof(uint64_t) * (size_t)grid * cells); sp.partials = partials->as<unsigned long long>(); }
   else { init_agg_cells(out_dev, n_groups, sh); sp.global_acc = (unsigned long long*)out_dev; }
+  SharedCellSink<SHAPE_Q1_ENCODED_PRICE>::Params cp{sp.partials, sp.global_acc, sp.n_groups, sp.copies, sp.oob, plan.shift};
   {
     ProfileScope ps(scope_name("fused_scan_ldsagg_static", "fused_scan_ldsagg_generic", static_id).c_str(), algo_bytes(sh, args), (uint64_t)args.n_rows);
-    switch (static_id) {
-      case SHAPE_Q1: launch_static<SHAPE_Q1, LdsAggSink>(wide, grid, lds, sh, args, sp); break;
-      case SHAPE_Q1_ENCODED: launch_static<SHAPE_Q1_ENCODED, LdsAggSink>(wide, grid, lds, sh, args, sp); break;
-      case SHAPE_Q1_ENCODED_PRICE: launch_static<SHAPE_Q1_ENCODED_PRICE, LdsAggSink>(wide, grid, lds, sh, args, sp); break;
-      default:
-        if (!jit::launch(sh, args, wide ? jit::LDSAGG_WIDE : jit::LDSAGG, &sp, grid, lds)) {
-          g_last_tile_rows.store(kTileRows, std::memory_order_relaxed);
-          const DynLaunch d = dyn_launch(sh, args, lds); PLX_LAUNCH_SCAN(DynProg, LdsAggSink, grid, d.lds, sh, d.args, sp);
-        }
-        break;
+    if (shared && static_id == SHAPE_Q1_ENCODED) {
+      SharedCellSink<SHAPE_Q1_ENCODED>::Params c15{cp.partials, cp.global_acc, cp.n_groups, cp.copies, cp.oob, cp.shift};
+      launch_static<SHAPE_Q1_ENCODED, SharedCellSink<SHAPE_Q1_ENCODED>>(wide, grid, lds, sh, args, c15);
+    } else if (shared && static_id == SHAPE_Q1_ENCODED_PRICE) {
+      launch_static<SHAPE_Q1_ENCODED_PRICE, SharedCellSink<SHAPE_Q1_ENCODED_PRICE>>(wide, grid, lds, sh, args, cp);
+    } else if (shared && jit::launch(sh, args, wide ? jit::LDSCELL_WIDE : jit::LDSCELL, &cp, grid, lds, code)) {
+    } else {
+      if (shared) {
+        shared = false; plan = cell_plan_from_code(sh, kIdentityCells);
+        copies = lds_agg_copies(n_groups, sh.n_aggs);
+        PLX_REQUIRE(copies > 0, PLX_ERR_INVALID, "fused_lds_agg: group table does not fit LDS");
+        sp.copies = copies; lds = (size_t)cells * copies * 8;
+      }
+      switch (static_id) {
+        case SHAPE_Q1: launch_static<SHAPE_Q1, LdsAggSink>(wide, grid, lds, sh, args, sp); break;
+        case SHAPE_Q1_ENCODED: launch_static<SHAPE_Q1_ENCODED, LdsAggSink>(wide, grid, lds, sh, args, sp); break;
+        case SHAPE_Q1_ENCODED_PRICE: launch_static<SHAPE_Q1_ENCODED_PRICE, LdsAggSink>(wide, grid, lds, sh, args, sp); break;
+        default:
+          if (!jit::launch(sh, args, wide ? jit::LDSAGG_WIDE : jit::LDSAGG, &sp, grid, lds)) {
+            g_last_tile_rows.store(kTileRows, std::memory_order_relaxed);
+            const DynLaunch d = dyn_launch(sh, args, lds); PLX_LAUNCH_SCAN(DynProg, LdsAggSink, grid, d.lds, sh, d.args, sp);
+          }
+          break;
+      }
     }
     PLX_HIP(hipGetLastError());
   }
+  g_last_lds_cells.store(plan.n_cells, std::memory_order_relaxed);
   if (use_partials) {
     hipLaunchKernelGGL(partials_finish_kernel, dim3(cells), dim3(kBlock), 0, stream(), sh, sp.partials, grid, cells, cells, (unsigned long long*)out_dev);
     PLX_HIP(hipGetLastError());
diff --git a/polars_amd/csrc/kernels_fused.hpp b/polars_amd/csrc/kernels_fused.hpp
--- a/polars_amd/csrc/kernels_fused.hpp
+++ b/polars_amd/csrc/kernels_fused.hpp
@@ -4,13 +4,19 @@
 
 #include "core.hpp"
 #include "fused.hpp"
+#include "fused_cells.hpp"
 
 namespace plx {
 namespace k {
 
 void fused_regagg(const fused::Shape& sh, const fused::Args& args, int static_id, uint64_t* out_host);
 int lds_agg_copies(int n_groups, int n_aggs);
-void fused_lds_agg(const fused::Shape& sh, const fused::Args& args, int n_groups, int static_id, uint64_t* out_dev, unsigned int* oob = nullptr );
+void fused_lds_agg(const fused::Shape& sh, const fused::Args& args, int n_groups, int static_id, uint64_t* out_dev, unsigned int* oob = nullptr ,
+                   const fused::CellPlan* cell_plan = nullptr );
+uint64_t lds_agg_wg_rows(int64_t n_rows);
+uint64_t lds_agg_wg_rows_of(int64_t n_rows, int grid, bool wide);
+int last_lds_cells();
+void set_shared_cells(bool on);
 
 bool wide_tiles_choice(const fused::Shape& sh, const fused::Args& args, bool compiled, bool knob_on);
 int last_scan_tile_rows();
```

Measured after the change: 444.5 billion rows/s (median of 6 runs). 1.12x the previous value.
